# JARVIS-MoCap/JARVIS-HybridNet

Measured on AMD Instinct MI355X. Metric: multi-view frames/s (12cam 1280x1024, 23kpt, 64^3 grid), higher is better.
Workload: dtype f32; 1 GPU; BASELINE configs[2]: HybridNet 12-camera 1280x1024, 23 kpts, 64^3 grid, small/small; cameras=12, joints=23, grid=64, streams=3, parallelism=single GPU, 3 time batches in flight on 3 HIP streams, hipgraph=False

## Files before the change

include/jarvis_hip.h:

```cpp
#ifndef JARVIS_HIP_H
#define JARVIS_HIP_H
#include <stdint.h>

#ifdef __cplusplus
extern "C" {
#endif

#define JH_ABI_VERSION 4

const char* jh_last_error(void);
int jh_abi_version(void);

#define JH_PRECISION_DEFAULT (-1)
#define JH_PRECISION_F32 0
#define JH_PRECISION_BF16X3 1
#define JH_PRECISION_BF16X3_WIDE 2
int jh_set_precision(int mode);
int jh_get_precision(void);

typedef struct jh_params jh_params;
int jh_params_create(jh_params** out);
int jh_params_set(jh_params* p, const char* key, const float* host, int64_t numel);
void jh_params_destroy(jh_params* p);

typedef struct jh_efftrack jh_efftrack;
int jh_efftrack_create(const jh_params* p, const char* prefix, int model_size, int joints, int n,
                       int h, int w, int want_res1, jh_efftrack** out);
int jh_efftrack_forward(jh_efftrack* net, const float* x_dev, float* res1_dev, float* res2_dev,
                        void* stream);
int64_t jh_efftrack_launches(const jh_efftrack* net);
void jh_efftrack_destroy(jh_efftrack* net);

typedef struct jh_v2v jh_v2v;
int jh_v2v_create(const jh_params* p, const char* prefix, int joints, int t, int g, jh_v2v** out);
int jh_v2v_forward(jh_v2v* net, const float* x_dev, float* y_dev, void* stream);
void jh_v2v_destroy(jh_v2v* net);

int64_t jh_reproject_workspace_bytes(int cams, int joints, int hs, int grid_size);
int jh_reproject_forward(const float* heatmaps_padded_dev, int cams, int joints, int hs,
                         const int32_t* center3d_dev, const int32_t* center_hm_dev,
                         const float* cam_dev, const float* intr_dev, const float* dist_dev,
                         int grid_size, float grid_spacing, float* vol_dev, int32_t* idx_dev,
                         void* workspace_dev, int64_t workspace_bytes, void* stream);

int64_t jh_softargmax_workspace_bytes(int t, int joints, int gh);
int jh_softargmax(const float* v2v_out_dev, int t, int joints, int gh, float grid_spacing,
                  float roi_cube_size, const int32_t* center3d_dev, float* heatmap_final_dev,
                  float* points_dev, float* conf_dev, void* workspace_dev, int64_t workspace_bytes,
                  void* stream);

int jh_reproject_point(const float* points_dev, int npoints, int cams, const float* cam_dev,
                       const float* intr_dev, const float* dist_dev, float* uv_dev, void* stream);
int64_t jh_reconstruct_workspace_bytes(int cams);
int jh_reconstruct_point(const float* points2d_dev, const float* maxvals_dev, int cams,
                         const float* cam_dev, const float* intr_dev, const float* dist_dev,
                         float* point3d_dev, void* workspace_dev, int64_t workspace_bytes,
                         void* stream);

typedef struct jh_predictor jh_predictor;
typedef struct {
  int32_t num_cameras, num_joints;
  int32_t center_size;
  int32_t bbox;
  float roi_cube_size;
  float grid_spacing;
  int32_t center_model, kp_model;
  int32_t img_h, img_w;
  int32_t time_batch;
  int32_t time_batch_3d;
  int32_t cam_lo, cam_n;
  float mean[3], std[3];
  int32_t precision;
} jh_predictor_config;

int jh_predictor_create(const jh_params* center_params, const jh_params* hybrid_params,
                        const jh_predictor_config* cfg, jh_predictor** out);
void jh_predictor_destroy(jh_predictor* pr);
int64_t jh_predictor_launches(const jh_predictor* pr);
int64_t jh_predictor_device_bytes(const jh_predictor* pr);
int jh_predictor_precision(const jh_predictor* pr);

int jh_predictor_set_calibration(jh_predictor* pr, const float* cam_dev, const float* intr_dev,
                                 const float* dist_dev, void* stream);
int jh_predictor_set_calibration_frames(jh_predictor* pr, const float* cam_dev ,
                                        const float* intr_dev , const float* dist_dev ,
                                        void* stream);

int jh_predictor_set_centers(jh_predictor* pr, const float* centers_dev , void* stream);

int jh_predictor_stage_center(jh_predictor* pr, const float* frames_dev, float* det_dev,
                              void* stream);
int jh_predictor_stage_keypoints(jh_predictor* pr, const float* frames_dev,
                                 const float* det_all_dev, float* heat_dev, void* stream);
int jh_predictor_stage_3d(jh_predictor* pr, const float* heat_all_dev, int t0, float* points_dev,
                          float* conf_dev, int32_t* valid_dev, void* stream);
int jh_predictor_stage_keypoints_gathered(jh_predictor* pr, const void* frames_dev, int frames_u8,
                                          const float* det_gathered_dev, int n_blocks,
                                          float* heat_dev, void* stream);
int jh_predictor_stage_3d_blocks(jh_predictor* pr, const float* heat_blocks_dev, int n_blocks,
                                 int frames_per_block, int t_off, int t0, float* points_dev,
                                 float* conf_dev, int32_t* valid_dev, void* stream);
int jh_predictor_forward(jh_predictor* pr, const float* frames_dev, float* points_dev,
                         float* conf_dev, int32_t* valid_dev, void* stream);
int jh_predictor_set_graph_replay(jh_predictor* pr, int on);
int jh_predictor_graph_replay(const jh_predictor* pr);
int jh_predictor_stage_center_u8(jh_predictor* pr, const uint8_t* frames_dev, float* det_dev,
                                 void* stream);
int jh_predictor_stage_keypoints_u8(jh_predictor* pr, const uint8_t* frames_dev,
                                    const float* det_all_dev, float* heat_dev, void* stream);
int jh_predictor_forward_u8(jh_predictor* pr, const uint8_t* frames_dev, float* points_dev,
                            float* conf_dev, int32_t* valid_dev, void* stream);

#define JH_FRAME_RGB_F32 0
#define JH_FRAME_BGR_U8 1
#define JH_FRAME_I420 2
#define JH_FRAME_NV12 3
int jh_predictor_forward_yuv(jh_predictor* pr, const uint8_t* frames_dev, int format, float* points_dev,
                             float* conf_dev, int32_t* valid_dev, void* stream);

#define JH_YUV_BT601 0
#define JH_YUV_BT709 1
#define JH_YUV_LIMITED 0
#define JH_YUV_FULL 1
typedef struct jh_yuv_surface {
  int64_t image_stride;
  int64_t y_offset, y_pitch;
  int64_t u_offset, v_offset;
  int64_t c_pitch;
  int32_t c_step;
  int32_t matrix;
  int32_t range;
  int32_t reserved;
} jh_yuv_surface;
int jh_yuv_surface_check(const jh_yuv_surface* surface, int h, int w);
int jh_predictor_forward_surface(jh_predictor* pr, const uint8_t* frames_dev, const jh_yuv_surface* surface,
                                 const uint8_t* mask_dev, float* points_dev, float* conf_dev, int32_t* valid_dev,
                                 void* stream);

#define JH_SENSOR_MONO 0
#define JH_SENSOR_RGGB 1
#define JH_SENSOR_BGGR 2
#define JH_SENSOR_GRBG 3
#define JH_SENSOR_GBRG 4
typedef struct jh_sensor_surface {
  int64_t image_stride;
  int64_t offset, pitch;
  int32_t pattern;
  int32_t reserved;
} jh_sensor_surface;
int jh_sensor_surface_check(const jh_sensor_surface* surface, int h, int w);
int jh_predictor_forward_sensor(jh_predictor* pr, const uint8_t* frames_dev, const jh_sensor_surface* surface,
                                const uint8_t* mask_dev, float* points_dev, float* conf_dev, int32_t* valid_dev,
                                void* stream);

int jh_predictor_debug(jh_predictor* pr, float* center3d_f_dev, int32_t* center3d_i_dev,
                       int32_t* center_hm_dev, float* det_dev, void* stream);

int jh_predictor_forward_masked(jh_predictor* pr, const void* frames_dev, int format, const uint8_t* mask_dev,
                                float* points_dev, float* conf_dev, int32_t* valid_dev, void* stream);
int jh_predictor_stage_keypoints_masked(jh_predictor* pr, const void* frames_dev, int format,
                                        const float* det_all_dev, const uint8_t* mask_dev, float* heat_dev,
                                        void* stream);
int jh_predictor_stage_3d_masked(jh_predictor* pr, const float* heat_all_dev, int t0, const uint8_t* mask_dev,
                                 float* points_dev, float* conf_dev, int32_t* valid_dev, void* stream);
int jh_predictor_debug_mask(jh_predictor* pr, int32_t* n_active_dev, int32_t* num_cams_detect_dev, void* stream);

int jh_predictor_views2d(jh_predictor* pr, const float* heat_all_dev, int t0, const float* points_dev,
                         const uint8_t* mask_dev, int32_t* points2d_dev, float* conf2d_dev, float* reproj_dev,
                         float* err_dev, uint8_t* used_dev, void* stream);

#define JH_FRAME_SURFACE  4
#define JH_FRAME_SENSOR   5
int jh_predictor_forward_images(jh_predictor* pr, const void* const* images_host, int n_images, int format,
                                const jh_yuv_surface* yuv, const jh_sensor_surface* sensor, const uint8_t* mask_dev,
                                float* points_dev, float* conf_dev, int32_t* valid_dev, void* stream);

int jh_predictor_hybridnet_forward(jh_predictor* pr, const float* crops_dev,
                                   const int32_t* center_hm_dev, const int32_t* center3d_dev,
                                   float* heatmap_final_dev, float* heatmaps_padded_dev,
                                   float* points_dev, float* conf_dev, void* stream);

typedef struct jh_predictor2d jh_predictor2d;
int jh_predictor2d_create(const jh_params* center_params, const jh_params* kp_params,
                          const jh_predictor_config* cfg, jh_predictor2d** out);
void jh_predictor2d_destroy(jh_predictor2d* pr);
int jh_predictor2d_forward(jh_predictor2d* pr, const float* frames_dev, int32_t* points_dev,
                           float* conf_dev, int32_t* valid_dev, void* stream);
int jh_predictor2d_forward_u8(jh_predictor2d* pr, const uint8_t* frames_dev, int32_t* points_dev,
                              float* conf_dev, int32_t* valid_dev, void* stream);

int jh_predictor2d_forward_yuv(jh_predictor2d* pr, const uint8_t* frames_dev, int format, int32_t* points_dev,
                               float* conf_dev, int32_t* valid_dev, void* stream);
int jh_predictor2d_forward_surface(jh_predictor2d* pr, const uint8_t* frames_dev, const jh_yuv_surface* surface,
                                   int32_t* points_dev, float* conf_dev, int32_t* valid_dev, void* stream);
int jh_predictor2d_forward_sensor(jh_predictor2d* pr, const uint8_t* frames_dev, const jh_sensor_surface* surface,
                                  int32_t* points_dev, float* conf_dev, int32_t* valid_dev, void* stream);

int jh_predictor2d_forward_images(jh_predictor2d* pr, const void* const* images_host, int n_images, int format,
                                  const jh_yuv_surface* yuv, const jh_sensor_surface* sensor,
                                  int32_t* points_dev, float* conf_dev, int32_t* valid_dev, void* stream);

int jh_profile_begin(void);
int jh_profile_end(int* n_records);
int jh_profile_get(int i, char* name, int name_cap, double* ms, double* flops, double* bytes);

int jh_op_conv(int nd, int kind, int k, int stride, int pad, int cin, int cout,
               const float* w_host, const float* b_host, const float* x_dev, int n, int d, int h,
               int w, const float* gate_dev, int norm_act, float* y_dev, void* stream);
int jh_op_depthwise(int k, int c, const float* w_host, const float* x_dev, int n, int h, int w,
                    int norm_act, float* y_dev, void* stream);
int jh_op_depthwise_pool(int k, int c, const float* w_host, const float* x_dev, int n, int h, int w,
                         float* y_dev, float* pool_dev, void* stream);

int jh_op_yuv420_to_bgr(const uint8_t* frames_dev, int format, int n, int h, int w, uint8_t* out_bgr_dev,
                        void* stream);
int jh_op_yuv_surface_to_bgr(const uint8_t* frames_dev, const jh_yuv_surface* surface, int n, int h, int w,
                             uint8_t* out_bgr_dev, void* stream);
int jh_op_sensor_to_bgr(const uint8_t* frames_dev, const jh_sensor_surface* surface, int n, int h, int w,
                        uint8_t* out_bgr_dev, void* stream);

int64_t jh_joint_argmax_all_workspace_bytes(int n, int hh, int wh, int jp);
int jh_op_joint_argmax_all(const float* heat_dev, int n, int hh, int wh, int j, int jp, int32_t* idx_dev,
                           float* max_dev, void* workspace_dev, int64_t workspace_bytes, void* stream);

int jh_op_bifpn_node(int n_in, const int* modes, const float* weights, int act, int n, int c, int cout,
                     int h, int w, const float* x0_dev, const float* x1_dev, const float* x2_dev,
                     const float* dw_host, const float* pw_host, const float* bias_host, float* y_dev,
                     void* stream);

#ifdef __cplusplus
}
#endif
#endif
```

jarvis-hybridnet_amd/_native.py:

```python
import ctypes
import math
import os
from typing import NamedTuple

import torch

_HERE = os.path.dirname(os.path.abspath(__file__))
LIB_PATH = os.environ.get("JH_LIBRARY_PATH") or os.path.join(_HERE, "libjarvis_hip.so")
_lib = None

c_void_p, c_int, c_float, c_int64 = ctypes.c_void_p, ctypes.c_int, ctypes.c_float, ctypes.c_int64
c_char_p = ctypes.c_char_p


class PredictorConfig(ctypes.Structure):
    _fields_ = [("num_cameras", ctypes.c_int32), ("num_joints", ctypes.c_int32),
                ("center_size", ctypes.c_int32), ("bbox", ctypes.c_int32),
                ("roi_cube_size", c_float), ("grid_spacing", c_float),
                ("center_model", ctypes.c_int32), ("kp_model", ctypes.c_int32),
                ("img_h", ctypes.c_int32), ("img_w", ctypes.c_int32),
                ("time_batch", ctypes.c_int32), ("time_batch_3d", ctypes.c_int32),
                ("cam_lo", ctypes.c_int32),
                ("cam_n", ctypes.c_int32), ("mean", c_float * 3), ("std", c_float * 3),
                ("precision", ctypes.c_int32)]


class YuvSurfaceStruct(ctypes.Structure):
    _fields_ = [("image_stride", ctypes.c_int64), ("y_offset", ctypes.c_int64), ("y_pitch", ctypes.c_int64),
                ("u_offset", ctypes.c_int64), ("v_offset", ctypes.c_int64), ("c_pitch", ctypes.c_int64),
                ("c_step", ctypes.c_int32), ("matrix", ctypes.c_int32), ("range", ctypes.c_int32),
                ("reserved", ctypes.c_int32)]


assert ctypes.sizeof(YuvSurfaceStruct) == 64


class SensorSurfaceStruct(ctypes.Structure):
    _fields_ = [("image_stride", ctypes.c_int64), ("offset", ctypes.c_int64), ("pitch", ctypes.c_int64),
                ("pattern", ctypes.c_int32), ("reserved", ctypes.c_int32)]


assert ctypes.sizeof(SensorSurfaceStruct) == 32

ABI_VERSION = 4
assert ctypes.sizeof(PredictorConfig) == 84

_WORKSPACES = {}


def workspace(nbytes, device):
    key = (str(device), torch.cuda.current_stream(device).cuda_stream)
    bufs = _WORKSPACES.setdefault(key, [])
    if not bufs or bufs[-1].numel() < nbytes:
        bufs.append(torch.empty((max(int(nbytes), 256),), dtype=torch.uint8, device=device))
    return bufs[-1]


_SIGS = {
    "jh_last_error": (c_char_p, []),
    "jh_abi_version": (c_int, []),
    "jh_set_precision": (c_int, [c_int]),
    "jh_get_precision": (c_int, []),
    "jh_params_create": (c_int, [ctypes.POINTER(c_void_p)]),
    "jh_params_set": (c_int, [c_void_p, c_char_p, c_void_p, c_int64]),
    "jh_params_destroy": (None, [c_void_p]),
    "jh_efftrack_create": (c_int, [c_void_p, c_char_p, c_int, c_int, c_int, c_int, c_int, c_int,
                                   ctypes.POINTER(c_void_p)]),
    "jh_efftrack_forward": (c_int, [c_void_p, c_void_p, c_void_p, c_void_p, c_void_p]),
    "jh_efftrack_launches": (c_int64, [c_void_p]),
    "jh_efftrack_destroy": (None, [c_void_p]),
    "jh_v2v_create": (c_int, [c_void_p, c_char_p, c_int, c_int, c_int, ctypes.POINTER(c_void_p)]),
    "jh_v2v_forward": (c_int, [c_void_p, c_void_p, c_void_p, c_void_p]),
    "jh_v2v_destroy": (None, [c_void_p]),
    "jh_reproject_workspace_bytes": (c_int64, [c_int, c_int, c_int, c_int]),
    "jh_reproject_forward": (c_int, [c_void_p, c_int, c_int, c_int, c_void_p, c_void_p, c_void_p,
                                     c_void_p, c_void_p, c_int, c_float, c_void_p, c_void_p,
                                     c_void_p, c_int64, c_void_p]),
    "jh_softargmax_workspace_bytes": (c_int64, [c_int, c_int, c_int]),
    "jh_softargmax": (c_int, [c_void_p, c_int, c_int, c_int, c_float, c_float, c_void_p, c_void_p,
                              c_void_p, c_void_p, c_void_p, c_int64, c_void_p]),
    "jh_reproject_point": (c_int, [c_void_p, c_int, c_int, c_void_p, c_void_p, c_void_p, c_void_p,
                                   c_void_p]),
    "jh_reconstruct_workspace_bytes": (c_int64, [c_int]),
    "jh_reconstruct_point": (c_int, [c_void_p, c_void_p, c_int, c_void_p, c_void_p, c_void_p,
                                     c_void_p, c_void_p, c_int64, c_void_p]),
    "jh_predictor_create": (c_int, [c_void_p, c_void_p, ctypes.POINTER(PredictorConfig),
                                    ctypes.POINTER(c_void_p)]),
    "jh_predictor_destroy": (None, [c_void_p]),
    "jh_predictor_set_graph_replay": (c_int, [c_void_p, c_int]),
    "jh_predictor_graph_replay": (c_int, [c_void_p]),
    "jh_predictor_launches": (c_int64, [c_void_p]),
    "jh_predictor_device_bytes": (c_int64, [c_void_p]),
    "jh_predictor_precision": (c_int, [c_void_p]),
    "jh_predictor_set_calibration": (c_int, [c_void_p, c_void_p, c_void_p, c_void_p, c_void_p]),
    "jh_predictor_set_calibration_frames": (c_int, [c_void_p, c_void_p, c_void_p, c_void_p, c_void_p]),
    "jh_predictor_set_centers": (c_int, [c_void_p, c_void_p, c_void_p]),
    "jh_predictor_stage_center": (c_int, [c_void_p, c_void_p, c_void_p, c_void_p]),
    "jh_predictor_stage_keypoints": (c_int, [c_void_p, c_void_p, c_void_p, c_void_p, c_void_p]),
    "jh_predictor_stage_3d": (c_int, [c_void_p, c_void_p, c_int, c_void_p, c_void_p, c_void_p,
                                      c_void_p]),
    "jh_predictor_stage_keypoints_gathered": (c_int, [c_void_p, c_void_p, c_int, c_void_p, c_int, c_void_p,
                                                      c_void_p]),
    "jh_predictor_stage_3d_blocks": (c_int, [c_void_p, c_void_p, c_int, c_int, c_int, c_int, c_void_p,
                                             c_void_p, c_void_p, c_void_p]),
    "jh_profile_begin": (c_int, []),
    "jh_profile_end": (c_int, [ctypes.POINTER(c_int)]),
    "jh_profile_get": (c_int, [c_int, c_char_p, c_int, ctypes.POINTER(ctypes.c_double),
                               ctypes.POINTER(ctypes.c_double), ctypes.POINTER(ctypes.c_double)]),
    "jh_predictor_forward": (c_int, [c_void_p, c_void_p, c_void_p, c_void_p, c_void_p, c_void_p]),
    "jh_predictor_stage_center_u8": (c_int, [c_void_p, c_void_p, c_void_p, c_void_p]),
    "jh_predictor_stage_keypoints_u8": (c_int, [c_void_p, c_void_p, c_void_p, c_void_p, c_void_p]),
    "jh_predictor_forward_u8": (c_int, [c_void_p, c_void_p, c_void_p, c_void_p, c_void_p, c_void_p]),
    "jh_predictor_forward_yuv": (c_int, [c_void_p, c_void_p, c_int, c_void_p, c_void_p, c_void_p, c_void_p]),
    "jh_yuv_surface_check": (c_int, [ctypes.POINTER(YuvSurfaceStruct), c_int, c_int]),
    "jh_predictor_forward_surface": (c_int, [c_void_p, c_void_p, ctypes.POINTER(YuvSurfaceStruct), c_void_p, c_void_p,
                                             c_void_p, c_void_p, c_void_p]),
    "jh_predictor2d_forward_surface": (c_int, [c_void_p, c_void_p, ctypes.POINTER(YuvSurfaceStruct), c_void_p,
                                               c_void_p, c_void_p, c_void_p]),
    "jh_op_yuv_surface_to_bgr": (c_int, [c_void_p, ctypes.POINTER(YuvSurfaceStruct), c_int, c_int, c_int, c_void_p,
                                         c_void_p]),
    "jh_sensor_surface_check": (c_int, [ctypes.POINTER(SensorSurfaceStruct), c_int, c_int]),
    "jh_predictor_forward_sensor": (c_int, [c_void_p, c_void_p, ctypes.POINTER(SensorSurfaceStruct), c_void_p, c_void_p,
                                            c_void_p, c_void_p, c_void_p]),
    "jh_predictor2d_forward_sensor": (c_int, [c_void_p, c_void_p, ctypes.POINTER(SensorSurfaceStruct), c_void_p,
                                              c_void_p, c_void_p, c_void_p]),
    "jh_op_sensor_to_bgr": (c_int, [c_void_p, ctypes.POINTER(SensorSurfaceStruct), c_int, c_int, c_int, c_void_p,
                                    c_void_p]),
    "jh_predictor_forward_masked": (c_int, [c_void_p, c_void_p, c_int, c_void_p, c_void_p, c_void_p, c_void_p,
                                            c_void_p]),
    "jh_predictor_forward_images": (c_int, [c_void_p, ctypes.POINTER(c_void_p), c_int, c_int,
                                            ctypes.POINTER(YuvSurfaceStruct), ctypes.POINTER(SensorSurfaceStruct),
                                            c_void_p, c_void_p, c_void_p, c_void_p, c_void_p]),
    "jh_predictor2d_forward_images": (c_int, [c_void_p, ctypes.POINTER(c_void_p), c_int, c_int,
                                              ctypes.POINTER(YuvSurfaceStruct), ctypes.POINTER(SensorSurfaceStruct),
                                              c_void_p, c_void_p, c_void_p, c_void_p]),
    "jh_predictor_stage_keypoints_masked": (c_int, [c_void_p, c_void_p, c_int, c_void_p, c_void_p, c_void_p,
                                                    c_void_p]),
    "jh_predictor_stage_3d_masked": (c_int, [c_void_p, c_void_p, c_int, c_void_p, c_void_p, c_void_p, c_void_p,
                                             c_void_p]),
    "jh_predictor_debug_mask": (c_int, [c_void_p, c_void_p, c_void_p, c_void_p]),
    "jh_predictor_views2d": (c_int, [c_void_p, c_void_p, c_int] + [c_void_p] * 8),
    "jh_joint_argmax_all_workspace_bytes": (c_int64, [c_int, c_int, c_int, c_int]),
    "jh_op_joint_argmax_all": (c_int, [c_void_p, c_int, c_int, c_int, c_int, c_int, c_void_p, c_void_p, c_void_p,
                                       c_int64, c_void_p]),
    "jh_predictor2d_create": (c_int, [c_void_p, c_void_p, ctypes.POINTER(PredictorConfig),
                                      ctypes.POINTER(c_void_p)]),
    "jh_predictor2d_destroy": (None, [c_void_p]),
    "jh_predictor2d_forward": (c_int, [c_void_p] * 6),
    "jh_predictor2d_forward_u8": (c_int, [c_void_p] * 6),
    "jh_predictor2d_forward_yuv": (c_int, [c_void_p, c_void_p, c_int, c_void_p, c_void_p, c_void_p, c_void_p]),
    "jh_predictor_debug": (c_int, [c_void_p, c_void_p, c_void_p, c_void_p, c_void_p, c_void_p]),
    "jh_predictor_hybridnet_forward": (c_int, [c_void_p] * 9),
    "jh_op_conv": (c_int, [c_int] * 7 + [c_void_p, c_void_p, c_void_p] + [c_int] * 4 +
                   [c_void_p, c_int, c_void_p, c_void_p]),
    "jh_op_depthwise": (c_int, [c_int, c_int, c_void_p, c_void_p, c_int, c_int, c_int, c_int,
                                c_void_p, c_void_p]),
    "jh_op_depthwise_pool": (c_int, [c_int, c_int, c_void_p, c_void_p, c_int, c_int, c_int, c_void_p, c_void_p,
                                     c_void_p]),
    "jh_op_yuv420_to_bgr": (c_int, [c_void_p, c_int, c_int, c_int, c_int, c_void_p, c_void_p]),
    "jh_op_bifpn_node": (c_int, [c_int, ctypes.POINTER(c_int), ctypes.POINTER(c_float), c_int, c_int, c_int,
                                 c_int, c_int, c_int, c_void_p, c_void_p, c_void_p, c_void_p, c_void_p,
                                 c_void_p, c_void_p, c_void_p]),
}


def symbols():
    return sorted(_SIGS)


def lib():
    global _lib
    if _lib is None:
        if not os.path.isfile(LIB_PATH):
            raise RuntimeError(
                "jarvis_hybridnet_amd: %s is missing -- build it with "
                "`python -c 'import __graft_entry__ as g; g.build()'` (hipcc, gfx950). "
                "There is no CPU fallback." % LIB_PATH)
        handle = ctypes.CDLL(LIB_PATH)
        for name, (res, args) in _SIGS.items():
            fn = getattr(handle, name)
            fn.restype, fn.argtypes = res, args
        if handle.jh_abi_version() != ABI_VERSION:
            raise RuntimeError("libjarvis_hip.so ABI version mismatch")
        _lib = handle
    return _lib


FRAME_CODES = {"rgb": 0, "bgr": 1, "i420": 2, "nv12": 3, "surface": 4, "sensor": 5}
FRAME_FORMATS = {k: FRAME_CODES[k] for k in ("bgr", "i420", "nv12")}
YUV_FORMATS = ("i420", "nv12")
FRAME_SURFACE, FRAME_SENSOR = FRAME_CODES["surface"], FRAME_CODES["sensor"]


class Frames(NamedTuple):
    fmt: int
    height: int
    width: int
    layout: object
    lead: tuple
    data: object = None
    images: object = None

    @property
    def device(self):
        return self.data.device if self.images is None else self.images[0].device


def yuv_format(name):
    if name not in YUV_FORMATS:
        raise ValueError("frame_format must be one of %s, got %r" % (list(YUV_FORMATS), name))
    return name


def surface(layout):
    if layout is None:
        raise ValueError("surface must be a YuvSurface or a SensorSurface, got None")
    return layout


def check_layout(layout, frame_format=None, hw=None):
    if layout is None:
        return None
    from .sensor_surface import SensorSurface
    from .yuv_surface import YuvSurface
    if not isinstance(layout, (YuvSurface, SensorSurface)):
        raise ValueError("frame_layout must be a YuvSurface or a SensorSurface or None, got %r"
                         % (type(layout).__name__,))
    if frame_format in YUV_FORMATS:
        raise ValueError("frame_layout describes the bytes itself: do not combine it with frame_format=%r"
                         % (frame_format,))
    if hw is not None and (layout.height, layout.width) != tuple(hw):
        raise ValueError("frame_layout is %d x %d; this predictor is %d x %d" % (layout.height, layout.width, *hw))
    return layout


def describe_shape(shape, dtype, lead, frame_format=None, frame_layout=None, hw=None, error=ValueError,
                   in_place=False, at_least=False):
    if frame_format is not None and frame_format not in FRAME_FORMATS:
        raise ValueError("frame_format must be one of %s or None, got %r" % (sorted(FRAME_FORMATS), frame_format))
    layout = check_layout(frame_layout, frame_format, hw)
    H, W = hw if hw is not None else ("H", "W")
    hint = ""
    if layout is not None:
        from .sensor_surface import SensorSurface
        kind, error = "sensor" if isinstance(layout, SensorSurface) else "surface", ValueError
        what = "frames of a %s (%simage_stride = %d bytes per image)" % (
            type(layout).__name__, "at least " if at_least else "", layout.image_stride)
        want, tail = torch.uint8, ("image_stride" if at_least else layout.image_stride,)
        H, W = layout.height, layout.width
    elif frame_format in YUV_FORMATS:
        if hw is not None and (H % 2 or W % 2):
            raise ValueError("YUV 4:2:0 frames need an even height and width; this predictor is %d x %d" % (H, W))
        kind, what, want = frame_format, "%s frames" % frame_format, torch.uint8
        tail = (H * 3 // 2, W) if hw is not None else ("3H/2", "W")
    elif dtype == torch.uint8:
        kind, what, want, tail = "bgr", "uint8 BGR frames", torch.uint8, (H, W, 3)
        if shape is not None and len(shape) == len(lead) + 2:
            hint = " (YUV 4:2:0 frames: pass frame_format='i420' or 'nv12')"
    elif frame_format == "bgr":
        raise error("frame_format 'bgr' needs uint8 %s frames; got dtype %s" % (_shape_text(lead, (H, W, 3)), dtype))
    elif dtype == torch.float32 or (not in_place and isinstance(dtype, torch.dtype)):
        kind, what, want, tail = "rgb", "fp32 RGB frames", dtype, (3, H, W)
    else:
        raise error("frames must be float32 RGB %s or uint8 BGR %s; got dtype %s"
                    % (_shape_text(lead, (3, H, W)), _shape_text(lead, (H, W, 3)), dtype))
    full = tuple(lead) + tail
    fits = shape is not None and dtype == want and len(shape) == len(full) and all(
        not isinstance(w, int) or int(g) == w for g, w in zip(shape, full))
    if fits and at_least and layout is not None:
        fits = int(shape[-1]) >= layout.image_stride
    if not fits:
        raise error("%s must be %s of shape %s; got %s%s" % (
            what, "uint8" if want == torch.uint8 else "float32", _shape_text(lead, tail),
            dtype if shape is None else "dtype %s, shape %s" % (dtype, tuple(shape)), hint))
    if kind in YUV_FORMATS and hw is None:
        rows, W = int(shape[-2]), int(shape[-1])
        if rows <= 0 or rows % 3 or W <= 0 or W % 2:
            raise ValueError("a YUV 4:2:0 image is (3H/2, W) bytes with H and W even; got (%d, %d)" % (rows, W))
        H = rows // 3 * 2
    elif hw is None and layout is None:
        H, W = (int(shape[-3]), int(shape[-2])) if kind == "bgr" else (int(shape[-2]), int(shape[-1]))
    return Frames(FRAME_CODES[kind], H, W, layout, tuple(int(n) for n in shape[:len(lead)]))


def _shape_text(lead, tail):
    return "(%s)" % ", ".join("*" if n is None else str(n) for n in tuple(lead) + tuple(tail))


def describe_frames(frames, lead, frame_format=None, frame_layout=None, hw=None, error=ValueError, in_place=False):
    shape, dtype = (frames.shape, frames.dtype) if torch.is_tensor(frames) else (None, type(frames).__name__)
    d = describe_shape(shape, dtype, lead, frame_format, frame_layout, hw, error, in_place)
    if not in_place:
        return d._replace(data=dev(frames, torch.uint8 if d.fmt else torch.float32))
    if not (frames.is_cuda and frames.is_contiguous()):
        raise RuntimeError("frames must be a contiguous CUDA (HIP) tensor")
    return d._replace(data=frames)


def frame_images(images, count, frame_format=None, frame_layout=None):
    lead = (count,) if isinstance(count, int) else tuple(count)
    count = math.prod(lead)
    if not isinstance(images, (list, tuple)) or len(images) != count or not images:
        raise ValueError("expected a sequence of %d images (one tensor per image); got %s" % (
            count, len(images) if isinstance(images, (list, tuple)) else type(images).__name__))
    for i, t in enumerate(images):
        if not torch.is_tensor(t):
            raise ValueError("image %d is a %s, not a tensor" % (i, type(t).__name__))
        if (t.shape, t.dtype, t.device) != (images[0].shape, images[0].dtype, images[0].device):
            raise ValueError("the images of a call have one shape, dtype and device: image %d is %s, image 0 is %s" % (
                i, (t.dtype, tuple(t.shape), str(t.device)),
                (images[0].dtype, tuple(images[0].shape), str(images[0].device))))
    d = describe_shape(images[0].shape, images[0].dtype, (), frame_format, frame_layout, in_place=True, at_least=True)
    for i, t in enumerate(images):
        if not t.is_contiguous():
            raise RuntimeError("image %d is not contiguous: the kernels read it in place" % i)
        if not t.is_cuda:
            raise RuntimeError("jarvis_hybridnet_amd needs CUDA (HIP) tensors; image %d is a CPU tensor" % i)
    return d._replace(lead=lead, images=list(images))


def forward_symbol(which, fmt, masked=False, per_image=False):
    if per_image:
        return which + "_forward_images"
    if fmt in (FRAME_SURFACE, FRAME_SENSOR):
        return which + ("_forward_surface" if fmt == FRAME_SURFACE else "_forward_sensor")
    if masked:
        return which + "_forward_masked"
    return which + ("_forward", "_forward_u8", "_forward_yuv", "_forward_yuv")[fmt]


def call_forward(which, handle, frames, mask, outs):
    masks = which == "jh_predictor"
    if mask is not None and not masks:
        raise ValueError("%s takes no camera mask" % which)
    name = forward_symbol(which, frames.fmt, mask is not None, frames.images is not None)
    struct = frames.layout.struct() if frames.layout is not None else None
    if frames.images is not None:
        table = (c_void_p * len(frames.images))(*(t.data_ptr() for t in frames.images))
        args = (table, len(frames.images), frames.fmt, struct if frames.fmt == FRAME_SURFACE else None,
                struct if frames.fmt == FRAME_SENSOR else None) + ((ptr(mask),) if masks else ())
    elif struct is not None:
        args = (ptr(frames.data), struct) + ((ptr(mask),) if masks else ())
    elif mask is not None:
        args = (ptr(frames.data), frames.fmt, ptr(mask))
    else:
        args = (ptr(frames.data),) + ((frames.fmt,) if frames.fmt >= FRAME_CODES["i420"] else ())
    check(getattr(lib(), name)(handle, *args, *(ptr(t) for t in outs), stream()))


def camera_mask(mask, shape, what="camera_mask"):
    if mask is None:
        return None
    if not torch.is_tensor(mask):
        try:
            mask = torch.as_tensor(mask)
        except Exception as e:
            raise ValueError("%s must be a bool or integer tensor or sequence of shape %s: %s" % (what, tuple(shape), e))
    if mask.dtype.is_floating_point or mask.dtype.is_complex:
        raise ValueError("%s must be bool or integer (nonzero = use the camera); got dtype %s" % (what, mask.dtype))
    if tuple(mask.shape) != tuple(shape):
        raise ValueError("%s must have shape %s; got %s" % (what, tuple(shape), tuple(mask.shape)))
    return (mask != 0).to(torch.uint8).contiguous()


_CALIB_TAILS = ((4, 3), (3, 3), (1, 5))


def calibration(calib, T, C):
    if not isinstance(calib, (list, tuple)) or len(calib) != 3 or not all(torch.is_tensor(t) for t in calib):
        raise ValueError("calibration is three tensors (cameraMatrices, intrinsicMatrices, distortionCoefficients); "
                         "got %s" % ([type(t).__name__ for t in calib] if isinstance(calib, (list, tuple))
                                     else type(calib).__name__))
    names = ("cameraMatrices", "intrinsicMatrices", "distortionCoefficients")
    forms = []
    for name, t, tail in zip(names, calib, _CALIB_TAILS):
        if not t.dtype.is_floating_point:
            raise ValueError("%s must be a floating-point tensor; got dtype %s" % (name, t.dtype))
        shape = tuple(int(n) for n in t.shape)
        if shape == (C,) + tail:
            forms.append("shared")
        elif shape == (T, C) + tail:
            forms.append("frames")
        else:
            raise ValueError("%s must have shape %s (shared by the frame sets) or %s (one per frame set); got %s"
                             % (name, (C,) + tail, (T, C) + tail, shape))
    if len(set(forms)) != 1:
        raise ValueError("the three calibration tensors are either all per camera (C, ...) or all per frame set "
                         "(T, C, ...); got %s" % ", ".join("%s: %s" % nf for nf in zip(names, forms)))
    return (forms[0],) + tuple(calib)


def centers(value, T):
    if value is None:
        return None
    want = "(%d, 3)" % T + (" or (3,)" if T == 1 else "")
    if not torch.is_tensor(value):
        try:
            value = torch.as_tensor(value)
        except Exception as e:
            raise ValueError("centers must be a real numeric tensor, array or sequence of shape %s: %s" % (want, e))
    if value.dtype == torch.bool or value.dtype.is_complex:
        raise ValueError("centers must have a real numeric dtype; got %s" % value.dtype)
    shape = tuple(int(n) for n in value.shape)
    if shape == (3,) and T == 1:
        value = value.unsqueeze(0)
    elif shape != (T, 3):
        raise ValueError("centers must have shape %s (world millimetres, one row per frame set); got %s" % (want, shape))
    return value.to(torch.float32).contiguous()


PRECISIONS = {"f32": 0, "bf16x3": 1, "bf16x3_wide": 2}
PRECISION_DEFAULT = -1


def precision_id(mode):
    if mode is None:
        return PRECISION_DEFAULT
    if mode not in PRECISIONS:
        raise ValueError("precision must be one of %s or None, got %r" % (sorted(PRECISIONS), mode))
    return PRECISIONS[mode]


def set_precision(mode):
    prev = get_precision()
    check(lib().jh_set_precision(PRECISIONS[mode]))
    return prev


def get_precision():
    return {v: k for k, v in PRECISIONS.items()}[lib().jh_get_precision()]


def check(rc):
    if rc != 0:
        raise RuntimeError("libjarvis_hip: " + lib().jh_last_error().decode())


def ptr(t):
    if t is None:
        return None
    assert t.is_contiguous(), "tensor must be contiguous"
    return t.data_ptr()


def dev(t, dtype=torch.float32):
    if not t.is_cuda:
        raise RuntimeError("jarvis_hybridnet_amd needs CUDA (HIP) tensors; got a CPU tensor")
    return t.to(dtype).contiguous()


def stream():
    return torch.cuda.current_stream().cuda_stream


class Params:

    def __init__(self, state_dict):
# ... 29 lines not shown
```

jarvis-hybridnet_amd/csrc/api.hip:

```cpp
#include <cstring>
#include <memory>
#include "../../include/jarvis_hip.h"
#include <cstdlib>
#include "nets.h"
#include "bifpn_node.h"
#include "camera_mask.h"
#include "views2d.h"

namespace jh {
static thread_local std::string g_err;
void set_error(const std::string& msg) { g_err = msg; }
}

using namespace jh;

struct jh_params { ParamMap map; };
struct jh_efftrack { EffTrackPlan plan; };
struct jh_v2v { V2VPlan plan; };

namespace {

struct Scratch {
  std::vector<void*> ptrs;
  ~Scratch() { for (void* p : ptrs) (void)hipFree(p); }
// ... 818 lines not shown
  return forward_impl(pr, frames_dev, fixed_source(kSrcBgrU8), points_dev, conf_dev, valid_dev, stream);
}

int jh_predictor_forward_yuv(jh_predictor* pr, const uint8_t* frames_dev, int format, float* points_dev,
                             float* conf_dev, int32_t* valid_dev, void* stream) {
  JH_REQUIRE(format == JH_FRAME_I420 || format == JH_FRAME_NV12, "jh_predictor_forward_yuv: format must be "
             "JH_FRAME_I420 or JH_FRAME_NV12");
  JH_REQUIRE(pr, "bad argument");
  FrameSource fs;
  if (frame_source(format, pr->cfg.img_h, pr->cfg.img_w, &fs)) return 1;
  return forward_impl(pr, frames_dev, fs, points_dev, conf_dev, valid_dev, stream);
}

int jh_yuv_surface_check(const jh_yuv_surface* surface, int h, int w) { return yuv_surface_check(surface, h, w); }

int jh_predictor_forward_surface(jh_predictor* pr, const uint8_t* frames_dev, const jh_yuv_surface* surface,
                                 const uint8_t* mask_dev, float* points_dev, float* conf_dev, int32_t* valid_dev,
                                 void* stream) {
  JH_REQUIRE(pr, "bad argument");
  FrameSource fs;
  if (frame_source(surface, pr->cfg.img_h, pr->cfg.img_w, &fs)) return 1;
  return forward_impl(pr, frames_dev, fs, points_dev, conf_dev, valid_dev, stream, mask_dev);
}

int jh_sensor_surface_check(const jh_sensor_surface* surface, int h, int w) {
  return sensor_surface_check(surface, h, w);
}

int jh_predictor_forward_sensor(jh_predictor* pr, const uint8_t* frames_dev, const jh_sensor_surface* surface,
                                const uint8_t* mask_dev, float* points_dev, float* conf_dev, int32_t* valid_dev,
                                void* stream) {
  JH_REQUIRE(pr, "bad argument");
  FrameSource fs;
  if (frame_source(surface, pr->cfg.img_h, pr->cfg.img_w, &fs)) return 1;
  return forward_impl(pr, frames_dev, fs, points_dev, conf_dev, valid_dev, stream, mask_dev);
}

int jh_predictor_forward_masked(jh_predictor* pr, const void* frames_dev, int format, const uint8_t* mask_dev,
                                float* points_dev, float* conf_dev, int32_t* valid_dev, void* stream) {
  JH_REQUIRE(pr, "bad argument");
  JH_REQUIRE(format >= JH_FRAME_RGB_F32 && format <= JH_FRAME_NV12, "jh_predictor_forward_masked: unknown frame format");
  FrameSource fs;
  if (frame_source(format, pr->cfg.img_h, pr->cfg.img_w, &fs)) return 1;
  return forward_impl(pr, frames_dev, fs, points_dev, conf_dev, valid_dev, stream, mask_dev);
}

int jh_predictor_forward_images(jh_predictor* pr, const void* const* images_host, int n_images, int format,
                                const jh_yuv_surface* yuv, const jh_sensor_surface* sensor, const uint8_t* mask_dev,
                                float* points_dev, float* conf_dev, int32_t* valid_dev, void* stream) {
  JH_REQUIRE(pr, "bad argument");
  JH_REQUIRE(pr->Cloc == pr->C && pr->cfg.cam_lo == 0, "forward needs all cameras local");
  FrameSource fs;
  if (images_source(format, yuv, sensor, pr->cfg.img_h, pr->cfg.img_w, &fs)) return 1;
  if (upload_images(pr->mem, &pr->frames_table, images_host, n_images, pr->T * pr->C, format,
                    static_cast<hipStream_t>(stream))) return 1;
  return forward_impl(pr, pr->frames_table, fs, points_dev, conf_dev, valid_dev, stream, mask_dev);
}

int jh_predictor_stage_keypoints_masked(jh_predictor* pr, const void* frames_dev, int format,
                                        const float* det_all_dev, const uint8_t* mask_dev, float* heat_dev,
                                        void* stream) {
  JH_REQUIRE(pr && mask_dev, "bad argument");
  JH_REQUIRE(format == JH_FRAME_RGB_F32 || format == JH_FRAME_BGR_U8, "masked stage 2: fp32 RGB or uint8 BGR frames");
  JH_REQUIRE(pr->Cloc == pr->C && pr->cfg.cam_lo == 0, "masked stage 2 needs all cameras local");
  pr->mask_cur = mask_dev;
  const int rc = stage_keypoints_impl(pr, frames_dev, fixed_source(format), det_all_dev, heat_dev, stream, 1, true);
  pr->mask_cur = nullptr;
  return rc;
}

int jh_predictor_stage_3d_masked(jh_predictor* pr, const float* heat_all_dev, int t0, const uint8_t* mask_dev,
                                 float* points_dev, float* conf_dev, int32_t* valid_dev, void* stream) {
  JH_REQUIRE(pr && mask_dev, "bad argument");
  JH_REQUIRE(pr->Cloc == pr->C && pr->cfg.cam_lo == 0, "masked stage 3 needs all cameras local");
  pr->mask_cur = mask_dev;
  const int rc = jh_predictor_stage_3d(pr, heat_all_dev, t0, points_dev, conf_dev, valid_dev, stream);
  pr->mask_cur = nullptr;
  return rc;
}

int jh_predictor_debug_mask(jh_predictor* pr, int32_t* n_active_dev, int32_t* num_cams_detect_dev, void* stream) {
  hipStream_t s = static_cast<hipStream_t>(stream);
  JH_REQUIRE(pr, "bad argument");
  const size_t T = pr->T;
  if (n_active_dev) JH_CHECK_HIP(hipMemcpyAsync(n_active_dev, pr->n_active, T * sizeof(int), hipMemcpyDeviceToDevice, s));
  if (num_cams_detect_dev) JH_CHECK_HIP(hipMemcpyAsync(num_cams_detect_dev, pr->n_detect, T * sizeof(int), hipMemcpyDeviceToDevice, s));
  return 0;
}

int jh_predictor_views2d(jh_predictor* pr, const float* heat_all_dev, int t0, const float* points_dev,
                         const uint8_t* mask_dev, int32_t* points2d_dev, float* conf2d_dev, float* reproj_dev,
                         float* err_dev, uint8_t* used_dev, void* stream) {
  hipStream_t s = static_cast<hipStream_t>(stream);
  JH_REQUIRE(pr && points_dev && points2d_dev && conf2d_dev && reproj_dev && err_dev && used_dev,
             "null pointer");
  JH_REQUIRE(t0 >= 0 && t0 + pr->T3 <= pr->T, "frame range of the 2D views");
  const int N = pr->T3 * pr->C;
  if (!heat_all_dev) {
    JH_REQUIRE(pr->Cloc == pr->C && pr->cfg.cam_lo == 0, "the predictor's own heat maps hold all cameras only when "
               "all cameras are local");
    heat_all_dev = pr->kp->heat.p + (size_t)t0 * pr->C * pr->Hh * pr->Hh * pr->Jp;
  }
  if (!pr->v2d_max) {
    hipStreamCaptureStatus cs = hipStreamCaptureStatusNone;
    (void)hipStreamIsCapturing(s, &cs);
    JH_REQUIRE(cs == hipStreamCaptureStatusNone, "the first jh_predictor_views2d call of a predictor allocates its "
               "workspace: make it outside a stream capture");
    const size_t n = joint_argmax_all_partials(N, pr->Hh, pr->Hh, pr->Jp);
    if (pr->mem.get(reinterpret_cast<void**>(&pr->v2d_max), n * sizeof(float))) return 1;
    if (pr->mem.get(reinterpret_cast<void**>(&pr->v2d_idx), n * sizeof(int))) return 1;
  }
  const double bytes = 4.0 * N * pr->Hh * pr->Hh * pr->Jp;
  JH_PROF("joint_argmax_all", 0.0, bytes,
          launch_joint_argmax_all(heat_all_dev, pr->v2d_max, pr->v2d_idx, N, pr->Hh, pr->Hh, pr->J, pr->Jp, s));
  const int slices = joint_argmax_all_shape(N, pr->Hh, pr->Hh, pr->Jp).slices;
  JH_PROF("views2d_final", 0.0, 8.0 * N * slices * pr->Jp + 24.0 * N * pr->J,
          launch_views2d_final(pr->v2d_max, pr->v2d_idx, pr->chm_cur() + (size_t)t0 * pr->C * 2, pr->valid_cur() + t0,
                               mask_dev ? mask_dev + (size_t)t0 * pr->C : nullptr, points_dev, pr->cam_at(t0),
                               pr->intr_at(t0), pr->dist_at(t0), pr->calib_fs, points2d_dev, conf2d_dev, reproj_dev,
                               err_dev, used_dev, pr->T3, pr->C,
                               pr->J, pr->Jp, pr->Hh, pr->Hh, pr->B / 2, s));
  return 0;
}

int jh_predictor_debug(jh_predictor* pr, float* center3d_f_dev, int32_t* center3d_i_dev,
                       int32_t* center_hm_dev, float* det_dev, void* stream) {
  hipStream_t s = static_cast<hipStream_t>(stream);
  const size_t T = pr->T, C = pr->C;
  if (center3d_f_dev) JH_CHECK_HIP(hipMemcpyAsync(center3d_f_dev, pr->c3f, T * 3 * sizeof(float), hipMemcpyDeviceToDevice, s));
  if (center3d_i_dev) JH_CHECK_HIP(hipMemcpyAsync(center3d_i_dev, pr->c3i_cur(), T * 3 * sizeof(int), hipMemcpyDeviceToDevice, s));
  if (center_hm_dev) JH_CHECK_HIP(hipMemcpyAsync(center_hm_dev, pr->chm_cur(), T * C * 2 * sizeof(int), hipMemcpyDeviceToDevice, s));
  if (det_dev) JH_CHECK_HIP(hipMemcpyAsync(det_dev, pr->det_all, T * C * 3 * sizeof(float), hipMemcpyDeviceToDevice, s));
  return 0;
}

int jh_predictor_hybridnet_forward(jh_predictor* pr, const float* crops_dev,
                                   const int32_t* center_hm_dev, const int32_t* center3d_dev,
                                   float* heatmap_final_dev, float* heatmaps_padded_dev,
                                   float* points_dev, float* conf_dev, void* stream) {
  hipStream_t s = static_cast<hipStream_t>(stream);
  JH_REQUIRE(pr->Cloc == pr->C && pr->T3 == pr->T, "hybridnet_forward needs all cameras local");
  JH_CHECK_HIP(hipMemcpyAsync(pr->chm_cur(), center_hm_dev, (size_t)pr->T * pr->C * 2 * sizeof(int), hipMemcpyDeviceToDevice, s));
  JH_CHECK_HIP(hipMemcpyAsync(pr->c3i_cur(), center3d_dev, (size_t)pr->T * 3 * sizeof(int), hipMemcpyDeviceToDevice, s));
  if (launch_to_channel_last(crops_dev, pr->kp->input, s)) return 1;
  pr->kp->stem_src.mode = 0;
  if (pr->kp->run(s)) return 1;
  if (heatmaps_padded_dev) {
    const Act& h = pr->kp->heat;
    const size_t total = (size_t)h.N * pr->J * pr->hs * pr->hs;
    int blocks = (int)((total + 255) / 256);
    if (blocks > 8192) blocks = 8192;
    hipLaunchKernelGGL(export_padded_kernel, dim3(blocks), dim3(256), 0, s, h.p, heatmaps_padded_dev,
                       h.N, pr->J, h.Cp, pr->Hh);
    JH_CHECK_HIP(hipGetLastError());
  }
  return pr->run_3d(pr->kp->heat.p, 0, heatmap_final_dev, points_dev, conf_dev, s);
}

}

struct jh_predictor2d {
  jh_predictor_config cfg{};
  int T = 0, J = 0, B = 0;
  std::unique_ptr<EffTrackPlan> center, kp;
  Scratch mem;
  float* det = nullptr;
  int *chm = nullptr, *valid = nullptr;
  const void** frames_table = nullptr;
};

extern "C" {

int jh_predictor2d_create(const jh_params* center_params, const jh_params* kp_params,
                          const jh_predictor_config* cfg, jh_predictor2d** out) {
  JH_REQUIRE(center_params && kp_params && cfg && out, "bad argument");
  std::unique_ptr<jh_predictor2d> pr(new jh_predictor2d());
  pr->cfg = *cfg;
  pr->T = cfg->time_batch; pr->J = cfg->num_joints; pr->B = cfg->bbox;
  JH_REQUIRE(pr->T >= 1, "batch");
  JH_REQUIRE(cfg->img_w >= pr->B + 1 && cfg->img_h >= pr->B + 1, "image smaller than the bounding box");
  JH_REQUIRE(cfg->precision >= JH_PRECISION_DEFAULT && cfg->precision <= JH_PRECISION_BF16X3_WIDE,
             "jh_predictor_config.precision: unknown mode");
  const int precision = cfg->precision == JH_PRECISION_DEFAULT ? precision_mode() : cfg->precision;
  pr->cfg.precision = precision;
  pr->center.reset(new EffTrackPlan());
  pr->center->precision = precision;
  if (pr->center->build(center_params->map, "", cfg->center_model, 1, pr->T, cfg->center_size,
                        cfg->center_size)) return 1;
  pr->kp.reset(new EffTrackPlan());
  pr->kp->precision = precision;
  if (pr->kp->build(kp_params->map, "", cfg->kp_model, pr->J, pr->T, pr->B, pr->B)) return 1;
  if (pr->mem.get(reinterpret_cast<void**>(&pr->det), (size_t)pr->T * 3 * sizeof(float))) return 1;
  if (pr->mem.get(reinterpret_cast<void**>(&pr->chm), (size_t)pr->T * 2 * sizeof(int))) return 1;
  if (pr->mem.get(reinterpret_cast<void**>(&pr->valid), (size_t)pr->T * sizeof(int))) return 1;
  JH_CHECK_HIP(hipDeviceSynchronize());
  *out = pr.release();
  return 0;
}

void jh_predictor2d_destroy(jh_predictor2d* pr) { delete pr; }

static int forward2d_impl(jh_predictor2d* pr, const void* frames, const FrameSource& fs, int32_t* points_dev,
                          float* conf_dev, int32_t* valid_dev, void* stream) {
  hipStream_t s = static_cast<hipStream_t>(stream);
  const auto& c = pr->cfg;
  const int S = c.center_size;
  JH_PROF("preprocess_resize", 0.0, (double)pr->T * S * S * (4.0 * fs.px_bytes() + 12.0),
          launch_preprocess_resize(frames, fs, pr->center->input.p, pr->T, c.img_h, c.img_w, S,
                                   c.mean, c.std, s, fs.per_image ? pr->frames_table : nullptr));
  if (pr->center->run(s)) return 1;
  const Act& h = pr->center->heat;
  JH_PROF("center_argmax", 0.0, 4.0 * pr->T * h.H * h.W,
          launch_center_argmax(h.p, pr->det, pr->T, h.H, h.W, h.Cp, s));
  const float sx = (float)c.img_w / (float)S, sy = (float)c.img_h / (float)S;
  if (launch_center2d(pr->det, pr->chm, pr->valid, pr->T, sx, sy, pr->B / 2, c.img_w, c.img_h, s))
    return 1;
  JH_PROF("preprocess_crop", 0.0, (double)pr->T * pr->B * pr->B * (fs.px_bytes() + 12.0),
          launch_preprocess_crop(frames, fs, pr->chm, pr->kp->input.p, pr->T, 1, 1, 0, c.img_h,
                                 c.img_w, pr->B, c.mean, c.std, s, fs.per_image ? pr->frames_table : nullptr));
  if (pr->kp->run(s)) return 1;
  const Act& k = pr->kp->heat;
  JH_PROF("joint_argmax", 0.0, 4.0 * pr->T * k.H * k.W * pr->J,
          launch_joint_argmax(k.p, pr->chm, points_dev, conf_dev, pr->T, pr->J, k.Cp, k.H, k.W,
                              pr->B / 2, s));
  if (valid_dev)
    JH_CHECK_HIP(hipMemcpyAsync(valid_dev, pr->valid, (size_t)pr->T * sizeof(int),
                                hipMemcpyDeviceToDevice, s));
  return 0;
}

int jh_predictor2d_forward(jh_predictor2d* pr, const float* frames_dev, int32_t* points_dev,
                           float* conf_dev, int32_t* valid_dev, void* stream) {
  return forward2d_impl(pr, frames_dev, fixed_source(kSrcRgbF32), points_dev, conf_dev, valid_dev, stream);
}
int jh_predictor2d_forward_u8(jh_predictor2d* pr, const uint8_t* frames_dev, int32_t* points_dev,
                              float* conf_dev, int32_t* valid_dev, void* stream) {
  return forward2d_impl(pr, frames_dev, fixed_source(kSrcBgrU8), points_dev, conf_dev, valid_dev, stream);
}

int jh_predictor2d_forward_yuv(jh_predictor2d* pr, const uint8_t* frames_dev, int format, int32_t* points_dev,
                               float* conf_dev, int32_t* valid_dev, void* stream) {
  JH_REQUIRE(format == JH_FRAME_I420 || format == JH_FRAME_NV12, "jh_predictor2d_forward_yuv: format must be "
             "JH_FRAME_I420 or JH_FRAME_NV12");
  JH_REQUIRE(pr, "bad argument");
  FrameSource fs;
  if (frame_source(format, pr->cfg.img_h, pr->cfg.img_w, &fs)) return 1;
  return forward2d_impl(pr, frames_dev, fs, points_dev, conf_dev, valid_dev, stream);
}

int jh_predictor2d_forward_surface(jh_predictor2d* pr, const uint8_t* frames_dev, const jh_yuv_surface* surface,
                                   int32_t* points_dev, float* conf_dev, int32_t* valid_dev, void* stream) {
  JH_REQUIRE(pr && frames_dev, "bad argument");
  FrameSource fs;
  if (frame_source(surface, pr->cfg.img_h, pr->cfg.img_w, &fs)) return 1;
  return forward2d_impl(pr, frames_dev, fs, points_dev, conf_dev, valid_dev, stream);
}

int jh_predictor2d_forward_sensor(jh_predictor2d* pr, const uint8_t* frames_dev, const jh_sensor_surface* surface,
                                  int32_t* points_dev, float* conf_dev, int32_t* valid_dev, void* stream) {
  JH_REQUIRE(pr && frames_dev, "bad argument");
  FrameSource fs;
  if (frame_source(surface, pr->cfg.img_h, pr->cfg.img_w, &fs)) return 1;
  return forward2d_impl(pr, frames_dev, fs, points_dev, conf_dev, valid_dev, stream);
}

int jh_predictor2d_forward_images(jh_predictor2d* pr, const void* const* images_host, int n_images, int format,
                                  const jh_yuv_surface* yuv, const jh_sensor_surface* sensor,
                                  int32_t* points_dev, float* conf_dev, int32_t* valid_dev, void* stream) {
  JH_REQUIRE(pr && points_dev && conf_dev, "bad argument");
  FrameSource fs;
  if (images_source(format, yuv, sensor, pr->cfg.img_h, pr->cfg.img_w, &fs)) return 1;
  if (upload_images(pr->mem, &pr->frames_table, images_host, n_images, pr->T, format,
                    static_cast<hipStream_t>(stream))) return 1;
  return forward2d_impl(pr, pr->frames_table, fs, points_dev, conf_dev, valid_dev, stream);
}

int jh_profile_begin(void) {
  Profiler& pf = profiler();
  pf.recs.clear();
  pf.on = true;
  return 0;
}
int jh_profile_end(int* n_records) {
  Profiler& pf = profiler();
  pf.on = false;
  if (pf.finish()) return 1;
  if (n_records) *n_records = (int)pf.recs.size();
  return 0;
}
int jh_profile_get(int i, char* name, int name_cap, double* ms, double* flops, double* bytes) {
  Profiler& pf = profiler();
  JH_REQUIRE(i >= 0 && i < (int)pf.recs.size(), "profile record index");
  const ProfRec& r = pf.recs[i];
  if (name && name_cap > 0) {
    strncpy(name, r.name.c_str(), name_cap - 1);
    name[name_cap - 1] = 0;
  }
  if (ms) *ms = r.ms;
  if (flops) *flops = r.flops;
  if (bytes) *bytes = r.bytes;
  return 0;
}

int jh_op_conv(int nd, int kind, int k, int stride, int pad, int cin, int cout,
               const float* w_host, const float* b_host, const float* x_dev, int n, int d, int h,
               int w, const float* gate_dev, int norm_act, float* y_dev, void* stream) {
  hipStream_t s = static_cast<hipStream_t>(stream);
  ConvDesc desc = kind == 0 ? conv_desc(nd, k, stride, pad, cin, cout)
                            : (kind == 1 ? deconv2d_k4s2p1_desc(cin, cout) : deconv3d_k2s2_desc(cin, cout));
  Scratch sc;
  Act x, y;
  if (nd == 2) d = 1;
  if (sc.act(n, d, h, w, cin, &x)) return 1;
  int Do, Ho, Wo;
  conv_out_shape(desc, d, h, w, &Do, &Ho, &Wo);
  if (sc.act(n, Do, Ho, Wo, cout, &y)) return 1;
  JH_CHECK_HIP(hipMemsetAsync(y.p, 0, y.bytes(), s));
  bool wino = kind == 0 && nd == 3 && k == 3 && stride == 1 && pad == 1 && !gate_dev;
  if (const char* e = getenv("JH_WINO")) wino = wino && atoi(e) != 0;
  const bool b3 = wino && precision_mode() >= 1;
  const bool d4b = kind == 1 && !b_host && norm_act < 0 && !gate_dev && precision_mode() >= 1 &&
                   deconv4_bf16x3_eligible(cout);
  const bool xb = kind == 0 && !wino && !gate_dev && conv_bf16x3_eligible(desc) && x.Cp == cpad(cin) &&
                  (precision_mode() == 2 || (precision_mode() == 1 && nd == 3));
  ConvWeights cw;
  if (xb) {
    if (pack_conv_bf16x3_weights(desc, w_host, b_host, &cw)) return 1;
  } else if (d4b) {
    if (pack_deconv4_bf16x3_weights(cin, cout, w_host, &cw)) return 1;
  } else if (b3) {
    if (pack_bf16x3_weights(cin, cout, w_host, b_host, &cw)) return 1;
  } else if (wino) {
    if (pack_wino_weights(cin, cout, w_host, b_host, &cw)) return 1;
  } else {
    if (pack_conv_weights(desc, w_host, b_host, kind != 0, &cw)) return 1;
  }
  double* stats = nullptr;
  float* gate_p = nullptr;
  int rc = 0;
  do {
    if (norm_act >= 0) {
      if ((rc = sc.get(reinterpret_cast<void**>(&stats), (size_t)n * y.Cp * kStatW * sizeof(double)))) break;
      if (hipMemsetAsync(stats, 0, (size_t)n * y.Cp * kStatW * sizeof(double), s) != hipSuccess) { rc = 1; break; }
    }
    if (gate_dev) {
      if ((rc = sc.get(reinterpret_cast<void**>(&gate_p), (size_t)n * x.Cp * sizeof(float)))) break;
      if (hipMemsetAsync(gate_p, 0, (size_t)n * x.Cp * sizeof(float), s) != hipSuccess) { rc = 1; break; }
      if (hipMemcpy2DAsync(gate_p, x.Cp * sizeof(float), gate_dev, cin * sizeof(float),
                           cin * sizeof(float), n, hipMemcpyDeviceToDevice, s) != hipSuccess) { rc = 1; break; }
    }
    if ((rc = launch_to_channel_last(x_dev, x, s))) break;
    if (xb) { if ((rc = launch_conv_bf16x3(desc, cw, x, y, stats, s, nullptr))) break; }
    else if (d4b) { if ((rc = launch_deconv4_bf16x3(cw, x, y, s, nullptr))) break; }
    else if (b3) { if ((rc = launch_conv3d_bf16x3(cw, x, y, stats, s, nullptr))) break; }
    else if (wino) { if ((rc = launch_conv3d_wino(cw, x, y, stats, s, nullptr, wino_variant_from_env()))) break; }
    else if ((rc = launch_conv(desc, cw, x, y, gate_p, stats, s))) break;
    if (norm_act >= 0 && (rc = launch_norm_apply(y, stats, 1e-5, norm_act, nullptr, nullptr, y.p, nullptr, s))) break;
    if ((rc = launch_from_channel_last(y, y_dev, s))) break;
    if (hipStreamSynchronize(s) != hipSuccess) { set_error("stream sync failed in jh_op_conv"); rc = 1; }
  } while (0);
  free_conv_weights(&cw);
  return rc;
}

int jh_op_depthwise(int k, int c, const float* w_host, const float* x_dev, int n, int h, int w,
                    int norm_act, float* y_dev, void* stream) {
  hipStream_t s = static_cast<hipStream_t>(stream);
  Scratch sc;
  Act x, y;
  if (sc.act(n, 1, h, w, c, &x)) return 1;
  if (sc.act(n, 1, h, w, c, &y)) return 1;
  std::vector<float> wt((size_t)k * k * x.Cp, 0.f);
  for (int ch = 0; ch < c; ++ch)
    for (int t = 0; t < k * k; ++t) wt[(size_t)t * x.Cp + ch] = w_host[(size_t)ch * k * k + t];
  float* wd; double* stats = nullptr;
  if (sc.get(reinterpret_cast<void**>(&wd), wt.size() * sizeof(float))) return 1;
  JH_CHECK_HIP(hipMemcpyAsync(wd, wt.data(), wt.size() * sizeof(float), hipMemcpyHostToDevice, s));
  if (norm_act >= 0) {
    if (sc.get(reinterpret_cast<void**>(&stats), (size_t)n * x.Cp * kStatW * sizeof(double))) return 1;
    JH_CHECK_HIP(hipMemsetAsync(stats, 0, (size_t)n * x.Cp * kStatW * sizeof(double), s));
  }
  if (launch_to_channel_last(x_dev, x, s)) return 1;
  if (launch_depthwise(x, wd, k, y.p, stats, s)) return 1;
  if (norm_act >= 0 && launch_norm_apply(y, stats, 1e-5, norm_act, nullptr, nullptr, y.p, nullptr, s)) return 1;
  if (launch_from_channel_last(y, y_dev, s)) return 1;
  JH_CHECK_HIP(hipStreamSynchronize(s));
  return 0;
}

int jh_op_yuv420_to_bgr(const uint8_t* frames_dev, int format, int n, int h, int w, uint8_t* out_bgr_dev,
                        void* stream) {
  hipStream_t s = static_cast<hipStream_t>(stream);
  JH_REQUIRE(frames_dev && out_bgr_dev, "null frame / output pointer");
  JH_REQUIRE(format == JH_FRAME_I420 || format == JH_FRAME_NV12, "jh_op_yuv420_to_bgr: format must be "
             "JH_FRAME_I420 or JH_FRAME_NV12");
  FrameSource fs;
  if (frame_source(format, h, w, &fs) || launch_frames_to_bgr(frames_dev, fs, out_bgr_dev, n, h, w, s)) return 1;
  JH_CHECK_HIP(hipStreamSynchronize(s));
  return 0;
}

int jh_op_yuv_surface_to_bgr(const uint8_t* frames_dev, const jh_yuv_surface* surface, int n, int h, int w,
                             uint8_t* out_bgr_dev, void* stream) {
  hipStream_t s = static_cast<hipStream_t>(stream);
  JH_REQUIRE(frames_dev && out_bgr_dev && n >= 1, "null frame / output pointer");
  FrameSource fs;
  if (frame_source(surface, h, w, &fs) || launch_frames_to_bgr(frames_dev, fs, out_bgr_dev, n, h, w, s)) return 1;
  JH_CHECK_HIP(hipStreamSynchronize(s));
  return 0;
}

int jh_op_sensor_to_bgr(const uint8_t* frames_dev, const jh_sensor_surface* surface, int n, int h, int w,
                        uint8_t* out_bgr_dev, void* stream) {
  hipStream_t s = static_cast<hipStream_t>(stream);
  JH_REQUIRE(frames_dev && out_bgr_dev && n >= 1, "null frame / output pointer");
  FrameSource fs;
  if (frame_source(surface, h, w, &fs) || launch_frames_to_bgr(frames_dev, fs, out_bgr_dev, n, h, w, s)) return 1;
  JH_CHECK_HIP(hipStreamSynchronize(s));
  return 0;
}

int jh_op_depthwise_pool(int k, int c, const float* w_host, const float* x_dev, int n, int h, int w,
                         float* y_dev, float* pool_dev, void* stream) {
  hipStream_t s = static_cast<hipStream_t>(stream);
  JH_REQUIRE(depthwise_can_pool(h, w), "jh_op_depthwise_pool: the image must be one 16 x 16 tile");
  Scratch sc;
  Act x, y;
  if (sc.act(n, 1, h, w, c, &x)) return 1;
  if (sc.act(n, 1, h, w, c, &y)) return 1;
  std::vector<float> wt((size_t)k * k * x.Cp, 0.f);
  for (int ch = 0; ch < c; ++ch)
    for (int t = 0; t < k * k; ++t) wt[(size_t)t * x.Cp + ch] = w_host[(size_t)ch * k * k + t];
  float* wd; double *stats = nullptr, *pool = nullptr;
  if (sc.get(reinterpret_cast<void**>(&wd), wt.size() * sizeof(float))) return 1;
  JH_CHECK_HIP(hipMemcpyAsync(wd, wt.data(), wt.size() * sizeof(float), hipMemcpyHostToDevice, s));
  const size_t nst = (size_t)n * x.Cp * kStatW, npl = (size_t)n * x.Cp * kLimbs;
  if (sc.get(reinterpret_cast<void**>(&stats), nst * sizeof(double))) return 1;
  if (sc.get(reinterpret_cast<void**>(&pool), npl * sizeof(double))) return 1;
  JH_CHECK_HIP(hipMemsetAsync(stats, 0, nst * sizeof(double), s));
  JH_CHECK_HIP(hipMemsetAsync(pool, 0, npl * sizeof(double), s));
  if (launch_to_channel_last(x_dev, x, s)) return 1;
  if (launch_depthwise(x, wd, k, y.p, stats, s, pool)) return 1;
  if (launch_from_channel_last(y, y_dev, s)) return 1;
  std::vector<double> hp(npl);
  JH_CHECK_HIP(hipMemcpyAsync(hp.data(), pool, npl * sizeof(double), hipMemcpyDeviceToHost, s));
  JH_CHECK_HIP(hipStreamSynchronize(s));
  std::vector<float> out((size_t)n * c);
  for (int i = 0; i < n; ++i)
    for (int ch = 0; ch < c; ++ch) {
      const double* q = hp.data() + ((size_t)i * x.Cp + ch) * kLimbs;
      out[(size_t)i * c + ch] = (float)((q[0] + q[1]) + q[2]);
    }
  JH_CHECK_HIP(hipMemcpy(pool_dev, out.data(), out.size() * sizeof(float), hipMemcpyHostToDevice));
  return 0;
}

static size_t carve_joint_argmax_all(Carver& c, int n, int hh, int wh, int jp, float** pmax, int** pidx) {
  const size_t k = joint_argmax_all_partials(n, hh, wh, jp);
  *pmax = c.take<float>(k);
  *pidx = c.take<int>(k);
  return c.off;
}

int64_t jh_joint_argmax_all_workspace_bytes(int n, int hh, int wh, int jp) {
  if (n < 1 || hh < 1 || wh < 1 || jp < 8 || jp % 8 || jp > 256) return 0;
  Carver c(nullptr, 0);
  float* pmax;
  int* pidx;
  return (int64_t)carve_joint_argmax_all(c, n, hh, wh, jp, &pmax, &pidx);
}

int jh_op_joint_argmax_all(const float* heat_dev, int n, int hh, int wh, int j, int jp, int32_t* idx_dev,
                           float* max_dev, void* workspace_dev, int64_t workspace_bytes, void* stream) {
  hipStream_t s = static_cast<hipStream_t>(stream);
  JH_REQUIRE(heat_dev && idx_dev && max_dev, "null pointer");
  JH_REQUIRE(n >= 1 && hh >= 1 && wh >= 1 && jp >= 8 && jp % 8 == 0 && jp <= 256 && j >= 1 && j <= jp,
             "jh_op_joint_argmax_all: shape");
  JH_REQUIRE(workspace_dev && workspace_bytes >= 0, "workspace (see jh_joint_argmax_all_workspace_bytes)");
  Carver c(workspace_dev, (size_t)workspace_bytes);
  float* pmax;
  int* pidx;
  carve_joint_argmax_all(c, n, hh, wh, jp, &pmax, &pidx);
  JH_REQUIRE(c.fits(), "workspace smaller than jh_joint_argmax_all_workspace_bytes()");
  const double bytes = 4.0 * n * hh * wh * jp;
  JH_PROF("joint_argmax_all", 0.0, bytes, launch_joint_argmax_all(heat_dev, pmax, pidx, n, hh, wh, j, jp, s));
  if (launch_joint_argmax_all_combine(pmax, pidx, idx_dev, max_dev, n, hh, wh, j, jp, s)) return 1;
  JH_CHECK_HIP(hipStreamSynchronize(s));
  return 0;
}


int jh_op_bifpn_node(int n_in, const int* modes, const float* weights, int act, int n, int c, int cout,
                     int h, int w, const float* x0_dev, const float* x1_dev, const float* x2_dev,
                     const float* dw_host, const float* pw_host, const float* bias_host, float* y_dev,
                     void* stream) {
  hipStream_t s = static_cast<hipStream_t>(stream);
  JH_REQUIRE(n_in >= 2 && n_in <= 3 && modes && weights && y_dev, "bad argument");
  const float* xs[3] = {x0_dev, x1_dev, x2_dev};
  Scratch sc;
  Act in[3], y;
  NodeArgs a{};
  a.n_in = n_in; a.act = act;
  for (int i = 0; i < n_in; ++i) {
    int hi = h, wi = w;
    if (modes[i] == FUSE_UP2) { hi = h / 2; wi = w / 2; }
    else if (modes[i] == FUSE_UP4) { hi = h / 4; wi = w / 4; }
    else if (modes[i] == FUSE_POOL2) { hi = h * 2; wi = w * 2; }
    if (sc.act(n, 1, hi, wi, c, &in[i])) return 1;
    if (launch_to_channel_last(xs[i], in[i], s)) return 1;
    const size_t px = (size_t)hi * wi;
    std::vector<float> host((size_t)n * c * px);
    JH_CHECK_HIP(hipMemcpyAsync(host.data(), xs[i], host.size() * sizeof(float), hipMemcpyDeviceToHost, s));
    JH_CHECK_HIP(hipStreamSynchronize(s));
    std::vector<double> st((size_t)n * in[i].Cp * kStatW, 0.0);
    for (int b = 0; b < n; ++b)
      for (int ch = 0; ch < c; ++ch) {
        double s1 = 0.0, s2 = 0.0;
        const float* p = host.data() + ((size_t)b * c + ch) * px;
        for (size_t k = 0; k < px; ++k) { s1 += p[k]; s2 += (double)p[k] * p[k]; }
        st[((size_t)b * in[i].Cp + ch) * kStatW + 1] = s1;
        st[((size_t)b * in[i].Cp + ch) * kStatW + kLimbs + 1] = s2;
      }
    double* std_dev;
    if (sc.get(reinterpret_cast<void**>(&std_dev), st.size() * sizeof(double))) return 1;
    JH_CHECK_HIP(hipMemcpyAsync(std_dev, st.data(), st.size() * sizeof(double), hipMemcpyHostToDevice, s));
    JH_CHECK_HIP(hipStreamSynchronize(s));
    a.in[i] = in[i].p; a.st[i] = std_dev; a.inv_cnt[i] = 1.f / (float)px; a.mode[i] = modes[i];
    a.w[i] = weights[i];
  }
  if (sc.act(n, 1, h, w, cout, &y)) return 1;
  JH_CHECK_HIP(hipMemsetAsync(y.p, 0, y.bytes(), s));
  const int Cp = in[0].Cp;
  std::vector<float> dwt((size_t)9 * Cp, 0.f);
  for (int ch = 0; ch < c; ++ch)
    for (int t = 0; t < 9; ++t) dwt[(size_t)t * Cp + ch] = dw_host[(size_t)ch * 9 + t];
  float* dwd;
  if (sc.get(reinterpret_cast<void**>(&dwd), dwt.size() * sizeof(float))) return 1;
  JH_CHECK_HIP(hipMemcpyAsync(dwd, dwt.data(), dwt.size() * sizeof(float), hipMemcpyHostToDevice, s));
  ConvWeights cw;
  if (pack_conv_weights(conv_desc(2, 1, 1, 0, c, cout), pw_host, bias_host, false, &cw)) return 1;
  double* ost;
  int rc = 0;
  do {
    if ((rc = sc.get(reinterpret_cast<void**>(&ost), (size_t)n * y.Cp * kStatW * sizeof(double)))) break;
    if (hipMemsetAsync(ost, 0, (size_t)n * y.Cp * kStatW * sizeof(double), s) != hipSuccess) { rc = 1; break; }
    a.dw = dwd; a.pw = cw.w; a.bias = cw.bias; a.y = y.p; a.stats = ost;
    a.N = n; a.H = h; a.W = w; a.Cp = Cp; a.cout_p = y.Cp; a.cout_p16 = cw.cout_p16;
    if ((rc = launch_bifpn_node(a, s))) break;
    if ((rc = launch_from_channel_last(y, y_dev, s))) break;
    if (hipStreamSynchronize(s) != hipSuccess) { set_error("stream sync failed in jh_op_bifpn_node"); rc = 1; }
  } while (0);
  free_conv_weights(&cw);
  return rc;
}

}
```

jarvis-hybridnet_amd/csrc/conv_host.hip:

```cpp
#include <vector>
#include <cstring>
#include <cstdlib>
#include <algorithm>
#include "conv_mfma.h"

namespace jh {

ConvDesc conv_desc(int nd, int k, int stride, int pad, int cin, int cout) {
  ConvDesc d{};
  d.nd = nd; d.k = k; d.stride = stride; d.ostride = 1; d.nphase = 1;
  d.cin = cin; d.cout = cout;
  d.phase[0].pad[0] = (nd == 3) ? pad : 0;
  d.phase[0].pad[1] = pad; d.phase[0].pad[2] = pad;
  d.phase[0].ooff[0] = d.phase[0].ooff[1] = d.phase[0].ooff[2] = 0;
  return d;
}

ConvDesc deconv2d_k4s2p1_desc(int cin, int cout) {
  ConvDesc d{};
  d.nd = 2; d.k = 2; d.stride = 1; d.ostride = 2; d.nphase = 4;
  d.cin = cin; d.cout = cout;
  for (int py = 0; py < 2; ++py)
    for (int px = 0; px < 2; ++px) {
      ConvPhase& p = d.phase[py * 2 + px];
      p.pad[0] = 0; p.pad[1] = py ? 0 : 1; p.pad[2] = px ? 0 : 1;
      p.ooff[0] = 0; p.ooff[1] = py; p.ooff[2] = px;
    }
  return d;
}

ConvDesc deconv3d_k2s2_desc(int cin, int cout) {
  ConvDesc d{};
  d.nd = 3; d.k = 1; d.stride = 1; d.ostride = 2; d.nphase = 8;
  d.cin = cin; d.cout = cout;
  for (int p = 0; p < 8; ++p) {
    d.phase[p].pad[0] = d.phase[p].pad[1] = d.phase[p].pad[2] = 0;
    d.phase[p].ooff[0] = (p >> 2) & 1; d.phase[p].ooff[1] = (p >> 1) & 1; d.phase[p].ooff[2] = p & 1;
  }
  return d;
}

void conv_out_shape(const ConvDesc& d, int D, int H, int W, int* Do, int* Ho, int* Wo) {
  if (d.ostride > 1) {
    *Do = (d.nd == 3) ? D * d.ostride : 1; *Ho = H * d.ostride; *Wo = W * d.ostride;
    return;
  }
  const int kd = (d.nd == 3) ? d.k : 1;
  *Do = (d.nd == 3) ? (D + 2 * d.phase[0].pad[0] - kd) / d.stride + 1 : 1;
  *Ho = (H + 2 * d.phase[0].pad[1] - d.k) / d.stride + 1;
  *Wo = (W + 2 * d.phase[0].pad[2] - d.k) / d.stride + 1;
}

static inline int deconv4_tap(int parity, int t) { return parity ? (t == 0 ? 2 : 0) : (t == 0 ? 3 : 1); }

int pack_conv_weights(const ConvDesc& d, const float* w, const float* b, bool transposed,
                      ConvWeights* out) {
  const int cin_p = cpad(d.cin);
  const int cout_p16 = round_up(d.cout, 16);
  const int kd = (d.nd == 3) ? d.k : 1;
  const int ntap = kd * d.k * d.k;
  const int nk8 = cin_p / 8, nb = cout_p16 / 16;
  const size_t phase_stride = (size_t)ntap * nk8 * nb * 128;
  std::vector<float> packed(phase_stride * d.nphase, 0.f);
  const bool paired = d.nd == 2 && d.ostride > 1 && deconv4_eligible(cin_p, cout_p16);
  const bool tap_paired = d.nd == 3 && d.k == 3 && d.stride == 2 && d.ostride == 1;
  if (tap_paired) packed.assign((size_t)((ntap + 1) / 2) * nk8 * nb * 256, 0.f);
  int skd, sk;
  if (d.ostride > 1 && d.nd == 2) { skd = 1; sk = 4; }
  else if (d.ostride > 1 && d.nd == 3) { skd = 2; sk = 2; }
  else { skd = kd; sk = d.k; }
  const size_t sktaps = (size_t)skd * sk * sk;
  for (int ph = 0; ph < d.nphase; ++ph) {
    for (int tz = 0; tz < kd; ++tz)
      for (int ty = 0; ty < d.k; ++ty)
        for (int tx = 0; tx < d.k; ++tx) {
          int sz = tz, sy = ty, sx = tx;
          if (d.ostride > 1 && d.nd == 2) {
            sy = deconv4_tap(d.phase[ph].ooff[1], ty);
            sx = deconv4_tap(d.phase[ph].ooff[2], tx);
          } else if (d.ostride > 1 && d.nd == 3) {
            sz = d.phase[ph].ooff[0]; sy = d.phase[ph].ooff[1]; sx = d.phase[ph].ooff[2];
          }
          const size_t stap = ((size_t)sz * sk + sy) * sk + sx;
          const int tap = (tz * d.k + ty) * d.k + tx;
          for (int ci = 0; ci < d.cin; ++ci)
            for (int co = 0; co < d.cout; ++co) {
              const float v = transposed ? w[((size_t)ci * d.cout + co) * sktaps + stap]
                                         : w[((size_t)co * d.cin + ci) * sktaps + stap];
              const int kc8 = ci / 8, kq = (ci % 8) / 2, j = ci % 2;
              const int nbk = co / 16, nn = co % 16;
              const int lane = kq * 16 + nn;
              if (tap_paired)
                packed[((((size_t)(tap / 2)) * nk8 + kc8) * nb + nbk) * 256 + lane * 4 + (tap & 1) * 2 + j] = v;
              else if (paired)
                packed[ph * phase_stride + (((size_t)tap * (nk8 / 2) + kc8 / 2) * nb + nbk) * 256 + lane * 4 + (kc8 & 1) * 2 + j] = v;
              else
                packed[ph * phase_stride + (((size_t)tap * nk8 + kc8) * nb + nbk) * 128 + lane * 2 + j] = v;
            }
        }
  }
  out->cin_p = cin_p; out->cout_p16 = cout_p16; out->paired = tap_paired ? 2 : (paired ? 1 : 0);
  out->phase_stride = tap_paired ? packed.size() : phase_stride;
  JH_CHECK_HIP(hipMalloc(&out->w, packed.size() * sizeof(float)));
  JH_CHECK_HIP(hipMemcpy(out->w, packed.data(), packed.size() * sizeof(float), hipMemcpyHostToDevice));
  out->bias = nullptr;
  if (b) {
    std::vector<float> bp(cout_p16, 0.f);
    std::memcpy(bp.data(), b, d.cout * sizeof(float));
    JH_CHECK_HIP(hipMalloc(&out->bias, bp.size() * sizeof(float)));
    JH_CHECK_HIP(hipMemcpy(out->bias, bp.data(), bp.size() * sizeof(float), hipMemcpyHostToDevice));
  }
  return 0;
}

void free_conv_weights(ConvWeights* w) {
  if (w->w) (void)hipFree(w->w);
  if (w->bias) (void)hipFree(w->bias);
  w->w = w->bias = nullptr;
}

static int pick_nr(int nb, int taps, bool heavy_staging, long units) {
  const double stage = (heavy_staging ? 1.5 : 0.5) / (double)taps;
  const long slots = 512;
  int best = 1;
  double best_cost = 1e30;
  for (int nr = 4; nr >= 1; --nr) {
    const long groups = (nb + nr - 1) / nr;
    const double cost = (double)std::max(units * groups, slots) * (stage + nr);
    if (cost < best_cost - 1e-9) { best_cost = cost; best = nr; }
  }
  return best;
}

int launch_conv(const ConvDesc& d, const ConvWeights& w, const Act& x, const Act& y,
                const float* gate, double* stats, hipStream_t s, const InNorm* in, const SeGate* se) {
  JH_REQUIRE(x.Cp == w.cin_p || (x.Cp == 4 && w.cin_p == 8), "conv input channel padding mismatch");
  JH_REQUIRE(y.Cp == cpad(d.cout), "conv output channel padding mismatch");
  JH_REQUIRE(x.N == y.N, "batch mismatch");
  ConvArgs a{};
  a.x = x.p; a.y = y.p; a.w = w.w; a.bias = w.bias; a.gate = gate; a.stats = stats;
  if (in && in->stats) {
    a.in_stats = in->stats; a.in_inv = in->inv; a.in_act = in->act;
    a.nrm_floats = 2 * w.cin_p;
  }
  if (gate) a.nrm_floats += w.cin_p;
  if (se && se->pool) {
    JH_REQUIRE(!gate, "either a gate tensor or a gate recipe");
    a.se = *se;
    a.nrm_floats += w.cin_p + round_up(se->C, 4) + round_up(se->S, 4);
  }
  a.N = x.N; a.Din = x.D; a.Hin = x.H; a.Win = x.W; a.cin_p = w.cin_p; a.in_px = x.Cp;
  a.Dy = y.D; a.Hy = y.H; a.Wy = y.W; a.cout_p = y.Cp; a.cout_p16 = w.cout_p16;
  a.ostride = d.ostride; a.nphase = d.nphase; a.phase_stride = w.phase_stride; a.paired = w.paired;
  for (int p = 0; p < d.nphase; ++p) a.phase[p] = d.phase[p];
  if (d.ostride > 1) { a.Dout = x.D; a.Hout = x.H; a.Wout = x.W; }
  else conv_out_shape(d, x.D, x.H, x.W, &a.Dout, &a.Hout, &a.Wout);
  int Do, Ho, Wo;
  conv_out_shape(d, x.D, x.H, x.W, &Do, &Ho, &Wo);
  JH_REQUIRE(Do == y.D && Ho == y.H && Wo == y.W, "conv output extent mismatch");
  const int taps = d.k * d.k * (d.nd == 3 ? d.k : 1);
  long units;
  if (d.nd == 2) units = (long)((a.Hout + 7) / 8) * ((a.Wout <= 8 ? a.Wout + 7 : a.Wout + 15) / (a.Wout <= 8 ? 8 : 16));
  else units = (long)((a.Dout + 1) / 2) * ((a.Hout + 3) / 4) * ((a.Wout + 15) / 16);
  units *= (long)a.nphase * a.N;
  const int nr = pick_nr(w.cout_p16 / 16, taps, (in && in->stats && in->act == ACT_SILU) || gate || (se && se->pool),
                         units);
  const size_t budget = 40 * 1024;
  if (d.nd == 2 && d.ostride == 2 && d.k == 2) {
    const int rc = launch_deconv4_fused(a, s);
    if (rc >= 0) return rc;
  }
  JH_REQUIRE((a.paired == 2) == (d.nd == 3 && d.k == 3 && d.stride == 2 && d.ostride == 1) && a.paired != 1,
             "paired weight layout without a kernel that reads it");
  if (conv_pw_direct_eligible(d, a)) return launch_conv_pw_direct(a, s);
  if (d.nd == 2) {
    const int small = (a.Wout <= 8) ? 1 : 0;
    const int big = (a.Wout >= 64 && a.Hout >= 64 && w.cin_p <= 32 && d.ostride == 1 && d.stride == 1 &&
               (d.k == 1 || d.k == 3)) ? 1 : 0;
    if (big) return conv_launch_2d_big(a, d.k, d.stride, nr, budget, s);
    if (d.k == 1 && d.stride == 1 && d.ostride == 1 && d.nphase == 1 && (a.Wout % 16 != 0 || a.Hout % 8 != 0) &&
        a.Hout * a.Wout >= 96 && a.Hin == a.Hout && a.Win == a.Wout && a.Hy == a.Hout && a.Wy == a.Wout) {
      ConvArgs f = a;
      f.Win = f.Wout = f.Wy = a.Hout * a.Wout;
      f.Hin = f.Hout = f.Hy = 1;
      return conv_launch_2d_k1_flat(f, nr, budget, s);
    }
    if (d.k == 1 && d.stride == 1) return conv_launch_2d_k1(a, nr, small, budget, s);
    if (d.k == 2 && d.stride == 1) return conv_launch_2d_k2(a, nr, small, budget, s);
    if (d.k == 3 && d.stride == 1 && d.ostride == 1 && a.Wout > 16 && a.Wout <= 20 && a.Hout <= 22 &&
        !d.latency_class)
      return conv_launch_2d_k3_w20(a, nr, std::max(budget, (size_t)64 * 1024), s);
    if (!d.latency_class && d.ostride == 1) {
      if (d.k == 5 && d.stride <= 2 && a.Wout > 32 && a.Wout <= 40)
        return conv_launch_2d_k5_w40(a, d.stride, nr, std::max(budget, (size_t)64 * 1024), s);
      if (d.k == 3 && d.stride == 2 && a.Wout > 16 && a.Wout <= 20 && a.Hout <= 22)
        return conv_launch_2d_k3s2_w20(a, nr, std::max(budget, (size_t)96 * 1024), s);
    }
    if (d.k == 3 && d.stride <= 2) return conv_launch_2d_k3(a, d.stride, nr, small, budget, s);
    if (d.k == 5 && d.stride <= 2) return conv_launch_2d_k5(a, d.stride, nr, small, budget, s);
  } else {
    const int nr_form = pick_nr(w.cout_p16 / 16, taps,
                                (in && in->stats && in->act == ACT_SILU) || gate || (se && se->pool), 1L << 40);
    const long tiles_big = (long)((a.Dout + 1) / 2) * ((a.Hout + 3) / 4) * ((a.Wout + 15) / 16) *
                           a.nphase * ((w.cout_p16 / 16 + nr_form - 1) / nr_form);
    int small = tiles_big < 16 ? 1 : 0;
    if (!small && d.k == 3 && d.stride == 1 && tiles_big >= 256) small = 2;
    if (d.k == 1 && d.stride == 1) return conv_launch_3d_k1(a, nr, small, budget, s);
    if (d.k == 2 && d.stride == 2) return conv_launch_3d_k2s2(a, nr, small, budget, s);
    if (d.k == 3 && d.stride <= 2) return conv_launch_3d_k3(a, d.stride, nr, small, budget, s);
  }
  JH_REQUIRE(false, "no convolution kernel for this (nd, k, stride)");
}

}
```

jarvis-hybridnet_amd/csrc/conv_mfma.h:

```cpp
#pragma once
#include <cstdlib>
#include <type_traits>
#include "jh_common.h"

namespace jh {

typedef float f32x4 __attribute__((ext_vector_type(4)));

template <int ND, int K, int STRIDE, int TZ, int TY, int TX>
struct ConvGeom {
  static constexpr int KD = (ND == 3) ? K : 1;
  static constexpr int KH = K, KW = K;
  static constexpr int NT = KD * KH * KW;
  static constexpr int PZ = (TZ - 1) * STRIDE + KD;
  static constexpr int PY = (TY - 1) * STRIDE + KH;
  static constexpr int PX = (TX - 1) * STRIDE + KW;
  static constexpr int NPIX = PZ * PY * PX;
  static constexpr int TM = TZ * TY * TX;
  static constexpr int MR = TM / 64;
  static constexpr int SPAD = (STRIDE == 1) ? 4 : 2;
  static_assert(TM % 64 == 0 || (TZ == 1 && TM / 64 >= 1), "tile must cover at least 64 pixels");
  static size_t lds_bytes(int kc) { return (size_t)NPIX * (kc + SPAD) * sizeof(float); }
};

// ... 280 lines not shown
      const float4 mu = *reinterpret_cast<const float4*>(nrm + c);
      const float4 rs = *reinterpret_cast<const float4*>(nrm + a.cin_p + c);
      v.x = (v.x - mu.x) * rs.x; v.y = (v.y - mu.y) * rs.y;
      v.z = (v.z - mu.z) * rs.z; v.w = (v.w - mu.w) * rs.w;
      if (a.in_act == ACT_RELU) {
        v.x = fmaxf(v.x, 0.f); v.y = fmaxf(v.y, 0.f); v.z = fmaxf(v.z, 0.f); v.w = fmaxf(v.w, 0.f);
      } else if (a.in_act == ACT_SILU) {
        v.x = silu_fast(v.x); v.y = silu_fast(v.y);
        v.z = silu_fast(v.z); v.w = silu_fast(v.w);
      }
    }
    if (gated) {
      const float4 g = *reinterpret_cast<const float4*>(gate_l + c);
      v.x *= g.x; v.y *= g.y; v.z *= g.z; v.w *= g.w;
    }
    return v;
  };
  if constexpr (PF) issue_pf(0);

  constexpr bool TAPPAIR = ND == 3 && K == 3 && STRIDE == 2;
  constexpr bool PIPE = (G::NT > 1) && (MR * NR * KC8 >= 12) && !TAPPAIR;
  constexpr bool BREG = !PIPE && (G::NT == 1 ? KC8 * NR <= 16 : G::NT * KC8 * NR <= 9);
  for (int c0 = 0; c0 < a.cin_p; c0 += KC) {
    float2 breg[BREG ? G::NT : 1][KC8][NR];
    if constexpr (BREG) {
#pragma unroll
      for (int tp = 0; tp < G::NT; ++tp)
#pragma unroll
        for (int k8 = 0; k8 < KC8; ++k8)
#pragma unroll
          for (int nr = 0; nr < NR; ++nr)
            breg[tp][k8][nr] = wload(tp * tap_stride + min((c0 >> 3) + k8, nkc8_total - 1) * nb16_total * 64, nr);
    }
    __syncthreads();
    if constexpr (PF) {
      const int mode = !a.in_stats ? 0 : (a.in_act == ACT_RELU ? 2 : (a.in_act == ACT_SILU ? 3 : 1));
      auto commit_pf = [&](auto mode_c) __attribute__((always_inline)) {
        constexpr int MODE = decltype(mode_c)::value;
        float4 mu0 = make_float4(0.f, 0.f, 0.f, 0.f), rs0 = make_float4(1.f, 1.f, 1.f, 1.f), gt0 = rs0;
        if (CQ) {
          const int cc = min(c0 + (tid % Q4) * 4, a.cin_p - 4);
          if (MODE != 0) {
            mu0 = *reinterpret_cast<const float4*>(nrm + cc);
            rs0 = *reinterpret_cast<const float4*>(nrm + a.cin_p + cc);
          }
          if (gated) gt0 = *reinterpret_cast<const float4*>(gate_l + cc);
        }
#pragma unroll
        for (int it = 0; it < ITER; ++it) {
          const int idx = tid + it * 256;
          if (idx < G::NPIX * Q4) {
            const int c4 = idx % Q4, pix = idx / Q4;
            float4 mu = mu0, rs = rs0, gt = gt0;
            if (!CQ) {
              const int cc = min(c0 + c4 * 4, a.cin_p - 4);
              if (MODE != 0) {
                mu = *reinterpret_cast<const float4*>(nrm + cc);
                rs = *reinterpret_cast<const float4*>(nrm + a.cin_p + cc);
              }
              if (gated) gt = *reinterpret_cast<const float4*>(gate_l + cc);
            }
            float4 v = pf[it];
            if (MODE != 0) {
              const float m = (pvo[it] < 0 || c0 + c4 * 4 >= a.in_px) ? 0.f : 1.f;
              v.x = (v.x - mu.x) * rs.x; v.y = (v.y - mu.y) * rs.y;
              v.z = (v.z - mu.z) * rs.z; v.w = (v.w - mu.w) * rs.w;
              if (MODE == 2) {
                v.x = fmaxf(v.x, 0.f); v.y = fmaxf(v.y, 0.f); v.z = fmaxf(v.z, 0.f); v.w = fmaxf(v.w, 0.f);
              } else if (MODE == 3) {
                v.x = silu_fast(v.x); v.y = silu_fast(v.y);
                v.z = silu_fast(v.z); v.w = silu_fast(v.w);
              }
              v.x *= m; v.y *= m; v.z *= m; v.w *= m;
            }
            if (gated) { v.x *= gt.x; v.y *= gt.y; v.z *= gt.z; v.w *= gt.w; }
            float2* dst = lds2 + pix * S2 + c4 * 2;
            dst[0] = make_float2(v.x, v.y);
            dst[1] = make_float2(v.z, v.w);
          }
        }
      };
      if (mode == 0) commit_pf(std::integral_constant<int, 0>{});
      else if (mode == 3) commit_pf(std::integral_constant<int, 3>{});
      else if (mode == 2) commit_pf(std::integral_constant<int, 2>{});
      else commit_pf(std::integral_constant<int, 1>{});
    } else {
      for (int idx = tid; idx < G::NPIX * Q4; idx += 256) {
        const float* src;
        const bool ok = patch_ok(idx, c0, &src);
        const int c4 = idx % Q4, pix = idx / Q4;
        float4 v = make_float4(0.f, 0.f, 0.f, 0.f);
        if (ok) v = finish(*reinterpret_cast<const float4*>(src), c0 + c4 * 4);
        float2* dst = lds2 + pix * S2 + c4 * 2;
        dst[0] = make_float2(v.x, v.y);
        dst[1] = make_float2(v.z, v.w);
      }
    }
    __syncthreads();
    if constexpr (PF) {
      if (c0 + KC < a.cin_p) issue_pf(c0 + KC);
    }

    if constexpr (PIPE) {
      int koff[KC8];
#pragma unroll
      for (int k8 = 0; k8 < KC8; ++k8)
        koff[k8] = min((c0 >> 3) + k8, nkc8_total - 1) * nb16_total * 64;
      float2 bn[KC8][NR], an[KC8][MR];
#pragma unroll
      for (int k8 = 0; k8 < KC8; ++k8) {
#pragma unroll
        for (int nr = 0; nr < NR; ++nr) bn[k8][nr] = wload(koff[k8], nr);
#pragma unroll
        for (int mr = 0; mr < MR; ++mr) an[k8][mr] = lds2[abase[mr] + k8 * 4];
      }
      for (int row = 0; row < G::KD * G::KH; ++row) {
        const int dz = row / G::KH, dy = row % G::KH;
        const int row_off = (dz * G::PY + dy) * G::PX * S2;
        const int nrow = min(row + 1, G::KD * G::KH - 1);
        const int next_row_off = ((nrow / G::KH) * G::PY + nrow % G::KH) * G::PX * S2;
#pragma unroll
        for (int dx = 0; dx < G::KW; ++dx) {
          const int tap = row * G::KW + dx;
          float2 bc[KC8][NR], ac[KC8][MR];
#pragma unroll
          for (int k8 = 0; k8 < KC8; ++k8) {
#pragma unroll
            for (int mr = 0; mr < MR; ++mr) ac[k8][mr] = an[k8][mr];
#pragma unroll
            for (int nr = 0; nr < NR; ++nr) bc[k8][nr] = bn[k8][nr];
          }
          const int wn = min(tap + 1, G::NT - 1) * tap_stride;
          const int noff = (dx + 1 < G::KW) ? row_off + (dx + 1) * S2 : next_row_off;
#pragma unroll
          for (int k8 = 0; k8 < KC8; ++k8) {
#pragma unroll
            for (int nr = 0; nr < NR; ++nr) bn[k8][nr] = wload(wn + koff[k8], nr);
#pragma unroll
            for (int mr = 0; mr < MR; ++mr) an[k8][mr] = lds2[abase[mr] + noff + k8 * 4];
          }
#pragma unroll
          for (int k8 = 0; k8 < KC8; ++k8) {
#pragma unroll
            for (int mr = 0; mr < MR; ++mr)
#pragma unroll
              for (int nr = 0; nr < NR; ++nr)
                acc[mr][nr] = __builtin_amdgcn_mfma_f32_16x16x4f32(ac[k8][mr].x, bc[k8][nr].x, acc[mr][nr], 0, 0, 0);
#pragma unroll
            for (int mr = 0; mr < MR; ++mr)
#pragma unroll
              for (int nr = 0; nr < NR; ++nr)
                acc[mr][nr] = __builtin_amdgcn_mfma_f32_16x16x4f32(ac[k8][mr].y, bc[k8][nr].y, acc[mr][nr], 0, 0, 0);
          }
          {
            constexpr int MPK = MR * NR * 2, LPK = NR + MR, EACH = MPK / LPK, REM = MPK - EACH * LPK;
#pragma unroll
            for (int k8 = 0; k8 < KC8; ++k8) {
#pragma unroll
              for (int j = 0; j < NR; ++j) {
                __builtin_amdgcn_sched_group_barrier(0x020, 1, 0);
                __builtin_amdgcn_sched_group_barrier(0x008, EACH, 0);
              }
#pragma unroll
              for (int j = 0; j < MR; ++j) {
                __builtin_amdgcn_sched_group_barrier(0x100, 1, 0);
                __builtin_amdgcn_sched_group_barrier(0x008, EACH, 0);
              }
              if (REM > 0) __builtin_amdgcn_sched_group_barrier(0x008, REM, 0);
            }
          }
        }
      }
    } else if constexpr (BREG) {
#pragma unroll
      for (int tp = 0; tp < G::NT; ++tp) {
        const int dz = tp / (G::KH * G::KW), dy = (tp / G::KW) % G::KH, dx = tp % G::KW;
        const int toff = ((dz * G::PY + dy) * G::PX + dx) * S2;
        float2 ac[KC8][MR];
#pragma unroll
        for (int k8 = 0; k8 < KC8; ++k8)
#pragma unroll
          for (int mr = 0; mr < MR; ++mr) ac[k8][mr] = lds2[abase[mr] + toff + k8 * 4];
#pragma unroll
        for (int k8 = 0; k8 < KC8; ++k8) {
#pragma unroll
          for (int mr = 0; mr < MR; ++mr)
#pragma unroll
            for (int nr = 0; nr < NR; ++nr)
              acc[mr][nr] = __builtin_amdgcn_mfma_f32_16x16x4f32(ac[k8][mr].x, breg[tp][k8][nr].x, acc[mr][nr], 0, 0, 0);
#pragma unroll
          for (int mr = 0; mr < MR; ++mr)
#pragma unroll
            for (int nr = 0; nr < NR; ++nr)
              acc[mr][nr] = __builtin_amdgcn_mfma_f32_16x16x4f32(ac[k8][mr].y, breg[tp][k8][nr].y, acc[mr][nr], 0, 0, 0);
        }
      }
    } else {
      int koff[KC8];
#pragma unroll
      for (int k8 = 0; k8 < KC8; ++k8)
        koff[k8] = min((c0 >> 3) + k8, nkc8_total - 1) * nb16_total * 64;
      if constexpr (TAPPAIR) {
        constexpr int NP = (G::NT + 1) / 2;
        typedef unsigned int wu4 __attribute__((ext_vector_type(4)));
        auto wload4 = [&](int idx4, int nr) __attribute__((always_inline)) -> float4 {
          const wu4 v = __builtin_amdgcn_raw_buffer_load_b128(wrs, wvo[nr] * 2, idx4 * 16, 0);
          return make_float4(__uint_as_float(v.x), __uint_as_float(v.y), __uint_as_float(v.z), __uint_as_float(v.w));
        };
        float4 b4[KC8][NR];
#pragma unroll
        for (int k8 = 0; k8 < KC8; ++k8)
#pragma unroll
          for (int nr = 0; nr < NR; ++nr) b4[k8][nr] = wload4(koff[k8], nr);
#pragma unroll
        for (int p = 0; p < NP; ++p) {
          constexpr int KHW = G::KH * G::KW;
          const int t0 = 2 * p, t1 = min(2 * p + 1, G::NT - 1);
          const int o0 = (((t0 / KHW) * G::PY + (t0 / G::KW) % G::KH) * G::PX + t0 % G::KW) * S2;
          const int o1 = (((t1 / KHW) * G::PY + (t1 / G::KW) % G::KH) * G::PX + t1 % G::KW) * S2;
          float2 a0[KC8][MR], a1[KC8][MR];
          float4 bc[KC8][NR];
#pragma unroll
          for (int k8 = 0; k8 < KC8; ++k8)
#pragma unroll
            for (int mr = 0; mr < MR; ++mr) {
              a0[k8][mr] = lds2[abase[mr] + o0 + k8 * 4];
              a1[k8][mr] = lds2[abase[mr] + o1 + k8 * 4];
            }
          const int wn = min(p + 1, NP - 1) * tap_stride;
#pragma unroll
          for (int k8 = 0; k8 < KC8; ++k8)
#pragma unroll
            for (int nr = 0; nr < NR; ++nr) {
              bc[k8][nr] = b4[k8][nr];
              b4[k8][nr] = wload4(wn + koff[k8], nr);
            }
#define JH_TP_STEP(AV, AC, BC)                                                                              \
  _Pragma("unroll") for (int mr = 0; mr < MR; ++mr) _Pragma("unroll") for (int nr = 0; nr < NR; ++nr)     \
    acc[mr][nr] = __builtin_amdgcn_mfma_f32_16x16x4f32(AV[k8][mr].AC, bc[k8][nr].BC, acc[mr][nr], 0, 0, 0);
#pragma unroll
          for (int k8 = 0; k8 < KC8; ++k8) { JH_TP_STEP(a0, x, x) JH_TP_STEP(a0, y, y) }
#pragma unroll
          for (int k8 = 0; k8 < KC8; ++k8) { JH_TP_STEP(a1, x, z) JH_TP_STEP(a1, y, w) }
#undef JH_TP_STEP
        }
      } else {
      float2 bn[KC8][NR];
#pragma unroll
      for (int k8 = 0; k8 < KC8; ++k8)
#pragma unroll
        for (int nr = 0; nr < NR; ++nr) bn[k8][nr] = wload(koff[k8], nr);
      int tap = 0;
      for (int dz = 0; dz < G::KD; ++dz)
        for (int dy = 0; dy < G::KH; ++dy) {
          const int row_off = (dz * G::PY + dy) * G::PX * S2;
#pragma unroll
          for (int dx = 0; dx < G::KW; ++dx, ++tap) {
            float2 bc[KC8][NR], ac[KC8][MR];
#pragma unroll
            for (int k8 = 0; k8 < KC8; ++k8)
#pragma unroll
              for (int mr = 0; mr < MR; ++mr) ac[k8][mr] = lds2[abase[mr] + row_off + dx * S2 + k8 * 4];
            const int wn = min(tap + 1, G::NT - 1) * tap_stride;
#pragma unroll
            for (int k8 = 0; k8 < KC8; ++k8)
#pragma unroll
              for (int nr = 0; nr < NR; ++nr) {
                bc[k8][nr] = bn[k8][nr];
                bn[k8][nr] = wload(wn + koff[k8], nr);
              }
#pragma unroll
            for (int k8 = 0; k8 < KC8; ++k8) {
#pragma unroll
              for (int mr = 0; mr < MR; ++mr)
#pragma unroll
                for (int nr = 0; nr < NR; ++nr)
                  acc[mr][nr] = __builtin_amdgcn_mfma_f32_16x16x4f32(ac[k8][mr].x, bc[k8][nr].x, acc[mr][nr], 0, 0, 0);
#pragma unroll
              for (int mr = 0; mr < MR; ++mr)
#pragma unroll
                for (int nr = 0; nr < NR; ++nr)
                  acc[mr][nr] = __builtin_amdgcn_mfma_f32_16x16x4f32(ac[k8][mr].y, bc[k8][nr].y, acc[mr][nr], 0, 0, 0);
            }
          }
        }
      }
    }
  }

  __syncthreads();
  EpilogueArgs e;
  e.y = a.y + (size_t)n * a.Dy * a.Hy * a.Wy * a.cout_p;
  e.bias = a.bias;
  e.stats = a.stats ? a.stats + (size_t)n * a.cout_p * kStatW : nullptr;
  e.Dout = a.Dout; e.Hout = a.Hout; e.Wout = a.Wout; e.Hy = a.Hy; e.Wy = a.Wy;
  e.cout_p = a.cout_p; e.cout_p16 = a.cout_p16; e.os = a.ostride; e.osz = a.ostride;
  e.offz = a.phase[ph].ooff[0]; e.offy = a.phase[ph].ooff[1]; e.offx = a.phase[ph].ooff[2];
  if (oz0 + TZ <= a.Dout && oy0 + TY <= a.Hout && ox0 + TX <= a.Wout)
    conv_epilogue<MR, NR, TY, TX, 4, true>(acc, e, lds, nb0, oz0, oy0, ox0, tid);
  else
    conv_epilogue<MR, NR, TY, TX>(acc, e, lds, nb0, oz0, oy0, ox0, tid);
}

inline int pick_kc8(int cin_p, size_t (*lds_bytes)(int), size_t budget) {
  int best = 1;
  double best_cost = 1e30;
  for (int k = 1; k <= 4; ++k) {
    if (lds_bytes(k * 8) > budget && k > 1) continue;
    const int chunks = (cin_p + k * 8 - 1) / (k * 8);
    const double cost = (double)chunks * k * 8 / cin_p + 0.02 * chunks;
    if (cost < best_cost - 1e-9) { best_cost = cost; best = k; }
  }
  return best;
}

template <int ND, int K, int STRIDE, int TZ, int TY, int TX, int NRV, int KC8V>
int launch_conv_inst(const ConvArgs& b, dim3 grid, hipStream_t s) {
  using G = ConvGeom<ND, K, STRIDE, TZ, TY, TX>;
  size_t lds = G::lds_bytes(KC8V * 8);
  const size_t red = (size_t)4 * 4 * 16 * 2 * sizeof(double);
  if (lds < red) lds = red;
  lds += (size_t)b.nrm_floats * sizeof(float);
  JH_REQUIRE(lds <= 160 * 1024, "conv patch does not fit LDS");
  auto kern = conv_mfma_kernel<ND, K, STRIDE, TZ, TY, TX, NRV, KC8V>;
  static bool big_lds_enabled = false;
  if (lds > 64 * 1024 && !big_lds_enabled) {
    JH_CHECK_HIP(hipFuncSetAttribute(reinterpret_cast<const void*>(kern),
                                     hipFuncAttributeMaxDynamicSharedMemorySize, 160 * 1024));
    big_lds_enabled = true;
  }
  ConvArgs c = b;
  c.fgx = make_fastdiv(grid.x); c.fgy = make_fastdiv(grid.y);
  c.ftx = make_fastdiv((b.Wout + TX - 1) / TX); c.fty = make_fastdiv((b.Hout + TY - 1) / TY);
  JH_REQUIRE(b.nphase == 1 || b.nphase == 4 || b.nphase == 8, "phase count");
  hipLaunchKernelGGL(kern, grid, dim3(256), lds, s, c);
  JH_CHECK_HIP(hipGetLastError());
  return 0;
}

template <int ND, int K, int STRIDE, int TZ, int TY, int TX>
int launch_conv_geom(const ConvArgs& a, int nr, size_t lds_budget, hipStream_t s) {
  using G = ConvGeom<ND, K, STRIDE, TZ, TY, TX>;
  ConvArgs b = a;
  const int kc8 = pick_kc8(b.cin_p, &G::lds_bytes, lds_budget);
  b.kc = kc8 * 8;
  const int tiles = ((b.Dout + TZ - 1) / TZ) * ((b.Hout + TY - 1) / TY) * ((b.Wout + TX - 1) / TX);
  const int nb = b.cout_p16 / 16;
  while (nr > 1 && (long)tiles * ((nb + nr - 1) / nr) * b.N * b.nphase <= 128) --nr;
  dim3 grid(tiles, (nb + nr - 1) / nr, b.N * b.nphase);
#define JH_CONV_CASE(NRV, KV) \
  if (nr == NRV && kc8 == KV) return launch_conv_inst<ND, K, STRIDE, TZ, TY, TX, NRV, KV>(b, grid, s);
#define JH_CONV_ROW(NRV) JH_CONV_CASE(NRV, 1) JH_CONV_CASE(NRV, 2) JH_CONV_CASE(NRV, 3) JH_CONV_CASE(NRV, 4)
  JH_CONV_ROW(1) JH_CONV_ROW(2) JH_CONV_ROW(3) JH_CONV_ROW(4)
#undef JH_CONV_ROW
#undef JH_CONV_CASE
  JH_REQUIRE(false, "bad (NR, KC8)");
}

bool conv_pw_direct_eligible(const ConvDesc& d, const ConvArgs& a);
int launch_conv_pw_direct(const ConvArgs& a, hipStream_t s);

int launch_deconv4_fused(const ConvArgs& a, hipStream_t s);
bool deconv4_eligible(int cin_p, int cout_p16);

int conv_launch_2d_k1(const ConvArgs& a, int nr, int small, size_t budget, hipStream_t s);
int conv_launch_2d_k1_flat(const ConvArgs& a, int nr, size_t budget, hipStream_t s);
int conv_launch_2d_k2(const ConvArgs& a, int nr, int small, size_t budget, hipStream_t s);
int conv_launch_2d_k3(const ConvArgs& a, int stride, int nr, int small, size_t budget, hipStream_t s);
int conv_launch_2d_k3_w20(const ConvArgs& a, int nr, size_t budget, hipStream_t s);
int conv_launch_2d_k5(const ConvArgs& a, int stride, int nr, int small, size_t budget, hipStream_t s);
int conv_launch_2d_k5_w40(const ConvArgs& a, int stride, int nr, size_t budget, hipStream_t s);
int conv_launch_2d_k3s2_w20(const ConvArgs& a, int nr, size_t budget, hipStream_t s);
int conv_launch_2d_big(const ConvArgs& a, int k, int stride, int nr, size_t budget, hipStream_t s);
int conv_launch_3d_k1(const ConvArgs& a, int nr, int small, size_t budget, hipStream_t s);
int conv_launch_3d_k2s2(const ConvArgs& a, int nr, int small, size_t budget, hipStream_t s);
int conv_launch_3d_k3(const ConvArgs& a, int stride, int nr, int small, size_t budget, hipStream_t s);

}
```

jarvis-hybridnet_amd/csrc/deconv4.hip:

```cpp
#include <type_traits>
#include "conv_mfma.h"

namespace jh {

namespace {
constexpr int kDTY = 8, kDTX = 16, kDPY = kDTY + 2, kDPX = kDTX + 2, kDNPIX = kDPY * kDPX;
constexpr int kDSPAD = 4;
}

template <int NRP, int KC8, bool TR>
__global__ __launch_bounds__(256) void deconv4_fused_kernel(const ConvArgs a) {
  constexpr int MR = 2, NR = 4 * NRP;
  constexpr int KC = KC8 * 8, S = KC + kDSPAD, S2 = S / 2, Q4 = KC / 4, KP = KC8 / 2;
  static_assert(KC8 % 2 == 0 && S2 % 2 == 0, "paired operand layout");
  extern __shared__ __attribute__((aligned(16))) float lds_all[];
  float* nrm = lds_all;
  float* lds = lds_all + a.nrm_floats;
  float2* lds2 = reinterpret_cast<float2*>(lds);
  const int tid = threadIdx.x;
  const int lane = tid & 63;
  const int wave = __builtin_amdgcn_readfirstlane(tid >> 6);
  const int mrow = lane & 15, kq = lane >> 4;
  const int tiles_x = (a.Win + kDTX - 1) / kDTX;
  const BlockId bid = xcd_block();
  const int tile_x = bid.x % tiles_x, tile_y = bid.x / tiles_x;
  const int n = bid.z;
  const int oy0 = tile_y * kDTY, ox0 = tile_x * kDTX;
  const int iy0 = oy0 - 1, ix0 = ox0 - 1;

  int abase[MR];
#pragma unroll
  for (int mr = 0; mr < MR; ++mr) {
    const int p = (wave * MR + mr) * 16 + mrow;
    abase[mr] = ((p / kDTX) * kDPX + p % kDTX) * S2 + kq * 2;
  }
  f32x4 acc[MR][NR];
#pragma unroll
  for (int mr = 0; mr < MR; ++mr)
#pragma unroll
    for (int nr = 0; nr < NR; ++nr) acc[mr][nr] = (f32x4){0.f, 0.f, 0.f, 0.f};

  if (a.in_stats) {
    for (int c = tid; c < a.cin_p; c += 256) {
      const double* st = a.in_stats + ((size_t)n * a.cin_p + c) * kStatW;
      const double mu = exact_read(st) * (double)a.in_inv;
      double var = exact_read(st + kLimbs) * (double)a.in_inv - mu * mu;
      if (var < 0.0) var = 0.0;
      nrm[c] = (float)mu;
      nrm[a.cin_p + c] = (float)(1.0 / sqrt(var + 1e-5));
    }
  }
  const float* __restrict__ xin = a.x + (size_t)n * a.Hin * a.Win * a.in_px;
  const int nkc8_total = a.cin_p >> 3;
  const float4* __restrict__ wbase = reinterpret_cast<const float4*>(a.w);
  const unsigned ulane = lane;
  const int tap_stride = (nkc8_total >> 1) * NRP * 64;
  const int phase_stride4 = (int)(a.phase_stride >> 2);

  constexpr int ITER = (kDNPIX * Q4 + 255) / 256;
  static_assert(256 % Q4 == 0, "one channel quad per thread");
  typedef float cf4 __attribute__((ext_vector_type(4)));
  float4 pf[ITER];
  int pvo[ITER];
  const __amdgpu_buffer_rsrc_t xrs = __builtin_amdgcn_make_buffer_rsrc(
      const_cast<float*>(xin), 0, (int)((size_t)a.Hin * a.Win * a.in_px * 4), 0x00020000);
  const int c4 = tid % Q4;
#pragma unroll
  for (int it = 0; it < ITER; ++it) {
    const int pix = tid / Q4 + it * (256 / Q4);
    const int px = pix % kDPX, py = pix / kDPX;
    const int iy = iy0 + py, ix = ix0 + px;
    const bool ok = pix < kDNPIX && iy >= 0 && iy < a.Hin && ix >= 0 && ix < a.Win;
    pvo[it] = ok ? ((iy * a.Win + ix) * a.in_px + c4 * 4) * 4 : (int)0x80000000;
  }
  auto issue_pf = [&](int c0) __attribute__((always_inline)) {
#pragma unroll
    for (int it = 0; it < ITER; ++it) {
      const int off = (c0 + c4 * 4 < a.in_px) ? pvo[it] : (int)0x80000000;
      const cf4 v = __builtin_bit_cast(cf4, __builtin_amdgcn_raw_buffer_load_b128(xrs, off, c0 * 4, 0));
      pf[it] = make_float4(v[0], v[1], v[2], v[3]);
    }
  };
  issue_pf(0);

  for (int c0 = 0; c0 < a.cin_p; c0 += KC) {
    __syncthreads();
    {
      const int mode = !a.in_stats ? 0 : (a.in_act == ACT_RELU ? 2 : (a.in_act == ACT_SILU ? 3 : 1));
      auto commit_pf = [&](auto mode_c) __attribute__((always_inline)) {
        constexpr int MODE = decltype(mode_c)::value;
        float4 mu = make_float4(0.f, 0.f, 0.f, 0.f), rs = make_float4(1.f, 1.f, 1.f, 1.f);
        const int cc = min(c0 + c4 * 4, a.cin_p - 4);
        if (MODE != 0) {
          mu = *reinterpret_cast<const float4*>(nrm + cc);
          rs = *reinterpret_cast<const float4*>(nrm + a.cin_p + cc);
        }
#pragma unroll
        for (int it = 0; it < ITER; ++it) {
          const int pix = tid / Q4 + it * (256 / Q4);
          if (pix < kDNPIX) {
            float4 v = pf[it];
            if (MODE != 0) {
              const float m = (pvo[it] < 0 || c0 + c4 * 4 >= a.in_px) ? 0.f : 1.f;
              v.x = (v.x - mu.x) * rs.x; v.y = (v.y - mu.y) * rs.y;
              v.z = (v.z - mu.z) * rs.z; v.w = (v.w - mu.w) * rs.w;
              if (MODE == 2) {
                v.x = fmaxf(v.x, 0.f); v.y = fmaxf(v.y, 0.f); v.z = fmaxf(v.z, 0.f); v.w = fmaxf(v.w, 0.f);
              } else if (MODE == 3) {
                v.x = silu_fast(v.x); v.y = silu_fast(v.y);
                v.z = silu_fast(v.z); v.w = silu_fast(v.w);
              }
              v.x *= m; v.y *= m; v.z *= m; v.w *= m;
            }
            float2* dst = lds2 + pix * S2 + (c4 >> 2) * 8 + (c4 & 1) * 4 + ((c4 >> 1) & 1);
            dst[0] = make_float2(v.x, v.y);
            dst[2] = make_float2(v.z, v.w);
          }
        }
      };
      if (mode == 0) commit_pf(std::integral_constant<int, 0>{});
      else if (mode == 3) commit_pf(std::integral_constant<int, 3>{});
      else if (mode == 2) commit_pf(std::integral_constant<int, 2>{});
      else commit_pf(std::integral_constant<int, 1>{});
    }
    __syncthreads();
    if (c0 + KC < a.cin_p) issue_pf(c0 + KC);

    int koff[KP];
#pragma unroll
    for (int k8 = 0; k8 < KP; ++k8) koff[k8] = min((c0 >> 4) + k8, (nkc8_total >> 1) - 1) * NRP * 64;
    auto wptr = [&](int g) __attribute__((always_inline)) -> const float4* {
      int idx = 0;
      for (int r = 0; r < 3; ++r)
        for (int s = 0; s < 3; ++s)
          for (int py = 0; py < 2; ++py)
            for (int px = 0; px < 2; ++px) {
              const int ty = r - py, tx = s - px;
              if (ty < 0 || ty > 1 || tx < 0 || tx > 1) continue;
              if (idx == g) return wbase + (size_t)(py * 2 + px) * phase_stride4 + (ty * 2 + tx) * tap_stride;
              ++idx;
            }
      return wbase;
    };
    float4 bq[3][KP][NRP];
#pragma unroll
    for (int g0 = 0; g0 < 2; ++g0) {
      const float4* w0 = wptr(g0) + ulane;
#pragma unroll
      for (int k8 = 0; k8 < KP; ++k8)
#pragma unroll
        for (int nr = 0; nr < NRP; ++nr) bq[g0][k8][nr] = w0[koff[k8] + nr * 64];
    }
    float4 an[KP][MR];
#pragma unroll
    for (int k8 = 0; k8 < KP; ++k8)
#pragma unroll
      for (int mr = 0; mr < MR; ++mr) an[k8][mr] = *reinterpret_cast<const float4*>(lds2 + abase[mr] + k8 * 8);
    int g = 0;
#pragma unroll
    for (int r = 0; r < 3; ++r)
#pragma unroll
      for (int s = 0; s < 3; ++s) {
        float4 ac[KP][MR];
#pragma unroll
        for (int k8 = 0; k8 < KP; ++k8)
#pragma unroll
          for (int mr = 0; mr < MR; ++mr) ac[k8][mr] = an[k8][mr];
        if (r * 3 + s + 1 < 9) {
          const int r1 = (r * 3 + s + 1) / 3, s1 = (r * 3 + s + 1) % 3;
#pragma unroll
          for (int k8 = 0; k8 < KP; ++k8)
#pragma unroll
            for (int mr = 0; mr < MR; ++mr)
              an[k8][mr] = *reinterpret_cast<const float4*>(lds2 + abase[mr] + (r1 * kDPX + s1) * S2 + k8 * 8);
        }
#pragma unroll
        for (int py = 0; py < 2; ++py)
#pragma unroll
          for (int px = 0; px < 2; ++px) {
            const int ty = r - py, tx = s - px;
            if (ty < 0 || ty > 1 || tx < 0 || tx > 1) continue;
            if (g + 2 < 16) {
              const float4* wn = wptr(g + 2) + ulane;
#pragma unroll
              for (int k8 = 0; k8 < KP; ++k8)
#pragma unroll
                for (int nr = 0; nr < NRP; ++nr) bq[(g + 2) % 3][k8][nr] = wn[koff[k8] + nr * 64];
            }
            __builtin_amdgcn_sched_barrier(0);
            const int ph = py * 2 + px;
#pragma unroll
            for (int k8 = 0; k8 < KP; ++k8) {
#define JH_D4_STEP(C)                                                                                          \
  _Pragma("unroll") for (int mr = 0; mr < MR; ++mr) _Pragma("unroll") for (int nr = 0; nr < NRP; ++nr)       \
    acc[mr][ph * NRP + nr] = TR ? __builtin_amdgcn_mfma_f32_16x16x4f32(bq[g % 3][k8][nr].C, ac[k8][mr].C,    \
                                                                       acc[mr][ph * NRP + nr], 0, 0, 0)       \
                                : __builtin_amdgcn_mfma_f32_16x16x4f32(ac[k8][mr].C, bq[g % 3][k8][nr].C,    \
                                                                       acc[mr][ph * NRP + nr], 0, 0, 0);
              JH_D4_STEP(x) JH_D4_STEP(y) JH_D4_STEP(z) JH_D4_STEP(w)
#undef JH_D4_STEP
            }
            __builtin_amdgcn_sched_barrier(0);
            ++g;
          }
      }
  }

  __syncthreads();
  EpilogueArgs e;
  e.y = a.y + (size_t)n * a.Hy * a.Wy * a.cout_p;
  e.bias = a.bias;
  e.stats = a.stats ? a.stats + (size_t)n * a.cout_p * kStatW : nullptr;
  e.Dout = 1; e.Hout = a.Hin; e.Wout = a.Win; e.Hy = a.Hy; e.Wy = a.Wy;
  e.cout_p = a.cout_p; e.cout_p16 = a.cout_p16; e.os = 2; e.osz = 2; e.offz = 0;
  const bool full = oy0 + kDTY <= a.Hin && ox0 + kDTX <= a.Win;
#pragma unroll
  for (int ph = 0; ph < 4; ++ph) {
    f32x4 pa[MR][NRP];
#pragma unroll
    for (int mr = 0; mr < MR; ++mr)
#pragma unroll
      for (int nr = 0; nr < NRP; ++nr) pa[mr][nr] = acc[mr][ph * NRP + nr];
    e.offy = ph >> 1; e.offx = ph & 1;
    if constexpr (TR) {
      if (full) conv_epilogue_tr<MR, NRP, kDTY, kDTX, true>(pa, e, 0, 0, oy0, ox0, tid);
      else conv_epilogue_tr<MR, NRP, kDTY, kDTX, false>(pa, e, 0, 0, oy0, ox0, tid);
    } else {
      if (full) conv_epilogue<MR, NRP, kDTY, kDTX, 4, true>(pa, e, lds, 0, 0, oy0, ox0, tid);
      else conv_epilogue<MR, NRP, kDTY, kDTX>(pa, e, lds, 0, 0, oy0, ox0, tid);
      if (e.stats && ph < 3) __syncthreads();
    }
  }
}

template <int NRP, int KC8, bool TR>
static int launch_deconv4_tr(const ConvArgs& a, hipStream_t s) {
  size_t lds = (size_t)kDNPIX * (KC8 * 8 + kDSPAD) * sizeof(float);
  const size_t red = (size_t)4 * 4 * 16 * 2 * sizeof(double);
  if (lds < red) lds = red;
  lds += (size_t)a.nrm_floats * sizeof(float);
  auto kern = deconv4_fused_kernel<NRP, KC8, TR>;
  const int tiles = ((a.Hin + kDTY - 1) / kDTY) * ((a.Win + kDTX - 1) / kDTX);
  hipLaunchKernelGGL(kern, dim3(tiles, 1, a.N), dim3(256), lds, s, a);
  JH_CHECK_HIP(hipGetLastError());
  return 0;
}

template <int NRP, int KC8>
static int launch_deconv4_inst(const ConvArgs& a, hipStream_t s) {
  if (!a.stats) return launch_deconv4_tr<NRP, KC8, true>(a, s);
  return launch_deconv4_tr<NRP, KC8, false>(a, s);
}

bool deconv4_eligible(int cin_p, int cout_p16) {
  return cout_p16 <= 32 && cin_p % 16 == 0;
}

int launch_deconv4_fused(const ConvArgs& a, hipStream_t s) {
  const int nrp = a.cout_p16 / 16;
  if (a.gate || nrp > 2 || a.nphase != 4) return -1;
  if (!a.paired) return -1;
  const int kc8 = a.cin_p % 32 == 0 ? 4 : 2;
  if (nrp == 2 && kc8 == 4) return launch_deconv4_inst<2, 4>(a, s);
  if (nrp == 2 && kc8 == 2) return launch_deconv4_inst<2, 2>(a, s);
  if (nrp == 1 && kc8 == 4) return launch_deconv4_inst<1, 4>(a, s);
  return launch_deconv4_inst<1, 2>(a, s);
}

}
```

jarvis-hybridnet_amd/csrc/jh_common.h:

```cpp
#pragma once
#include <hip/hip_runtime.h>
#include <cstdlib>
#include <cstdint>
#include <cstdio>
#include <string>
#include <vector>

namespace jh {

constexpr int kWave = 64;

#define JH_ENV_KNOB(name) ([]() -> int { static const int v = [] { const char* e = getenv(name); return e ? atoi(e) : -1; }(); return v; }())

inline int round_up(int v, int m) { return (v + m - 1) / m * m; }
inline int cpad(int c) { return round_up(c, 8); }

void set_error(const std::string& msg);
#define JH_CHECK_HIP(expr)                                                     \
  do {                                                                         \
    hipError_t _e = (expr);                                                    \
    if (_e != hipSuccess) {                                                    \
      jh::set_error(std::string(#expr) + ": " + hipGetErrorString(_e));        \
      return 1;                                                                \
    }                                                                          \
  } while (0)
#define JH_REQUIRE(cond, msg)                                                  \
  do {                                                                         \
    if (!(cond)) {                                                             \
      jh::set_error(std::string("requirement failed: ") + #cond + " (" + msg + \
                    ")");                                                      \
      return 1;                                                                \
    }                                                                          \
  } while (0)

struct Act {
  float* p = nullptr;
  int N = 0, D = 1, H = 0, W = 0, C = 0, Cp = 0;
  size_t pixels() const { return (size_t)D * H * W; }
  size_t elems() const { return (size_t)N * pixels() * Cp; }
  size_t bytes() const { return elems() * sizeof(float); }
};

struct HeatLayout {
  int cams_per_block = 0;
  size_t block_stride = 0, frame_stride = 0;
};

enum ActKind { ACT_NONE = 0, ACT_RELU = 1, ACT_SILU = 2 };

struct ProfRec { std::string name; double flops, bytes; hipEvent_t e0, e1; float ms; };
struct Profiler {
  bool on = false;
  std::vector<ProfRec> recs;
  void begin(const std::string& name, double flops, double bytes, hipStream_t s);
  void end(hipStream_t s);
  int finish();
};
Profiler& profiler();

struct ConvPhase {
  int pad[3];
  int ooff[3];
};

struct ConvDesc {
  int nd;
  int k;
  int stride;
  int ostride;
  int nphase;
  ConvPhase phase[8];
  int cin, cout;
  int latency_class;
};

struct ConvWeights {
  float* w = nullptr;
  int paired = 0;
  float* bias = nullptr;
  size_t phase_stride = 0;
  int cin_p = 0, cout_p16 = 0;
};

struct FastDiv {
  unsigned mul = 1, shift = 0, d = 1;
};
inline FastDiv make_fastdiv(unsigned d) {
  FastDiv f;
  f.d = d;
  unsigned l = 0;
  while ((1ull << l) < d) ++l;
  f.shift = l;
  f.mul = (unsigned)((((1ull << l) - d) << 32) / d + 1);
  return f;
}

struct SeGate {
  const double* pool = nullptr;
  const float *wr = nullptr, *br = nullptr, *we = nullptr, *be = nullptr;
  int C = 0, S = 0;
  float inv_hw = 0.f;
};

struct ConvArgs {
  const float* x;
  float* y;
  const float* w;
  const float* bias;
  const float* gate;
  SeGate se;
  const double* in_stats;
  float in_inv;
  int in_act;
  int nrm_floats;
  double* stats;
  int N, Din, Hin, Win, cin_p;
  int Dout, Hout, Wout;
  int Dy, Hy, Wy, cout_p;
  int cout_p16;
  int kc;
  int in_px;
  int ostride, nphase;
  int paired = 0;
  FastDiv fgx, fgy, ftx, fty;
  size_t phase_stride;
  ConvPhase phase[8];
};

int pack_conv_weights(const ConvDesc& d, const float* w_host, const float* b_host,
                      bool transposed, ConvWeights* out);
void free_conv_weights(ConvWeights* w);

struct InNorm {
  const double* stats = nullptr;
  float inv = 0.f;
  int act = 0;
};
int launch_conv(const ConvDesc& d, const ConvWeights& w, const Act& x, const Act& y,
                const float* gate, double* stats, hipStream_t s, const InNorm* in = nullptr,
                const SeGate* se = nullptr);
void conv_out_shape(const ConvDesc& d, int D, int H, int W, int* Do, int* Ho, int* Wo);

ConvDesc conv_desc(int nd, int k, int stride, int pad, int cin, int cout);
ConvDesc deconv2d_k4s2p1_desc(int cin, int cout);
ConvDesc deconv3d_k2s2_desc(int cin, int cout);

int launch_norm_apply(const Act& x, const double* stats, double eps, int act,
                      const float* r1, const float* r2, float* y, double* pool,
                      hipStream_t s, const double* r1_stats = nullptr, int min_block_kb = 0);
int launch_se_gate(const double* pool, int N, int C, int Cp, int S, float inv_hw,
                   const float* wr, const float* br, const float* we, const float* be,
                   float* gate, hipStream_t s);
bool depthwise_can_pool(int H, int W);
int launch_depthwise(const Act& x, const float* w, int k, float* y, double* stats,
                     hipStream_t s, double* pool = nullptr);
enum FuseMode { FUSE_SAME = 0, FUSE_UP2 = 1, FUSE_UP4 = 2, FUSE_POOL2 = 3 };
struct FuseArgs {
  const float* in[3];
  int mode[3];
  float w[3];
  int n_in;
  int act;
};
int launch_fuse(const FuseArgs& f, const Act& out, hipStream_t s);
int launch_maxpool2(const Act& x, float* y, hipStream_t s);

struct BlockId { unsigned x, y, z; };

constexpr int kLimbs = 3;
constexpr int kStatW = 2 * kLimbs;
#if defined(__HIPCC__)
__device__ __forceinline__ void exact_add(double* dst, double p) {
  const double h = rint(p * 0x1p-16) * 0x1p16;
  const double r = p - h;
  const double m = rint(r * 0x1p20) * 0x1p-20;
  const double l = rint((r - m) * 0x1p56) * 0x1p-56;
  if (h != 0.0) unsafeAtomicAdd(dst + 0, h);
  if (m != 0.0) unsafeAtomicAdd(dst + 1, m);
  if (l != 0.0) unsafeAtomicAdd(dst + 2, l);
}
__device__ __forceinline__ double exact_read(const double* src) { return (src[0] + src[1]) + src[2]; }
__device__ __forceinline__ void stat_add(double* st, float s1, float s2) {
  exact_add(st, (double)s1);
  exact_add(st + kLimbs, (double)s2);
}
__device__ __forceinline__ void exact_add_rounded(double* dst, double p) {
  const double a = fabs(p);
  double q;
  int slot;
  if (a < 0x1p5) { q = rint(p * 0x1p35) * 0x1p-35; slot = 2; }
  else if (a < 0x1p15) { q = rint(p * 0x1p25) * 0x1p-25; slot = 1; }
  else { q = rint(p * 0x1p15) * 0x1p-15; slot = 0; }
  if (q != 0.0) unsafeAtomicAdd(dst + slot, q);
}
__device__ __forceinline__ void stat_add(double* st, double s1, double s2) {
  exact_add_rounded(st, s1);
  exact_add_rounded(st + kLimbs, s2);
}
__device__ __forceinline__ void stat_acc(double& s1, double& s2, float v) {
  const double d = (double)v;
  s1 += d;
  s2 = fma(d, d, s2);
}
#endif

#if defined(__HIPCC__)
__device__ __forceinline__ unsigned xcd_linear(unsigned L, unsigned total) {
  const unsigned q = total >> 3, r = total & 7u, x = L & 7u, s = L >> 3;
  return x < r ? x * (q + 1) + s : r * (q + 1) + (x - r) * q + s;
}
__device__ __forceinline__ unsigned fd_div(unsigned x, const FastDiv& f) { return (__umulhi(x, f.mul) + x) >> f.shift; }
__device__ __forceinline__ BlockId xcd_block(const FastDiv& fgx, const FastDiv& fgy) {
  const unsigned gx = gridDim.x, gy = gridDim.y, gz = gridDim.z;
  const unsigned L = blockIdx.x + gx * (blockIdx.y + gy * blockIdx.z);
  const unsigned l = xcd_linear(L, gx * gy * gz);
  BlockId b;
  const unsigned l1 = fd_div(l, fgx);
  b.x = l - l1 * gx;
  b.z = fd_div(l1, fgy);
  b.y = l1 - b.z * gy;
  return b;
}
__device__ __forceinline__ BlockId xcd_block() {
  const unsigned gx = gridDim.x, gy = gridDim.y, gz = gridDim.z;
  const unsigned L = blockIdx.x + gx * (blockIdx.y + gy * blockIdx.z);
  unsigned l = xcd_linear(L, gx * gy * gz);
  BlockId b;
  b.x = l % gx; l /= gx;
  b.y = l % gy;
  b.z = l / gy;
  return b;
}
#endif

#if defined(__HIPCC__)
__device__ __forceinline__ float sum_xor16(float s) {
  const auto r = __builtin_amdgcn_permlane16_swap(__float_as_uint(s), __float_as_uint(s), false, false);
  return __uint_as_float(r[0]) + __uint_as_float(r[1]);
}
__device__ __forceinline__ float sum_xor32(float s) {
  const auto r = __builtin_amdgcn_permlane32_swap(__float_as_uint(s), __float_as_uint(s), false, false);
  return __uint_as_float(r[0]) + __uint_as_float(r[1]);
}
__device__ __forceinline__ double sum_xor16(double s) {
  const unsigned lo = (unsigned)__double2loint(s), hi = (unsigned)__double2hiint(s);
  const auto a = __builtin_amdgcn_permlane16_swap(lo, lo, false, false);
  const auto b = __builtin_amdgcn_permlane16_swap(hi, hi, false, false);
  return __hiloint2double((int)b[0], (int)a[0]) + __hiloint2double((int)b[1], (int)a[1]);
}
__device__ __forceinline__ double sum_xor32(double s) {
  const unsigned lo = (unsigned)__double2loint(s), hi = (unsigned)__double2hiint(s);
  const auto a = __builtin_amdgcn_permlane32_swap(lo, lo, false, false);
  const auto b = __builtin_amdgcn_permlane32_swap(hi, hi, false, false);
  return __hiloint2double((int)b[0], (int)a[0]) + __hiloint2double((int)b[1], (int)a[1]);
}
__device__ __forceinline__ float silu_fast(float v) { return v * __builtin_amdgcn_rcpf(1.f + __expf(-v)); }
#endif

struct NodeArgs;
int launch_bifpn_node(const NodeArgs& a, hipStream_t s);
int pack_wino_weights(int cin, int cout, const float* w, const float* b, ConvWeights* out);
int wino_variant_from_env();
int launch_conv3d_wino(const ConvWeights& w, const Act& x, const Act& y, double* stats, hipStream_t s,
                       const InNorm* in, int variant = 4, const int* tables = nullptr);
int pack_bf16x3_weights(int cin, int cout, const float* w, const float* b, ConvWeights* out);
int launch_conv3d_bf16x3(const ConvWeights& w, const Act& x, const Act& y, double* stats, hipStream_t s,
                         const InNorm* in);
int pack_deconv4_bf16x3_weights(int cin, int cout, const float* w, ConvWeights* out);
bool deconv4_bf16x3_eligible(int cout);
int launch_deconv4_bf16x3(const ConvWeights& w, const Act& x, const Act& y, hipStream_t s, const InNorm* in);
bool conv_bf16x3_eligible(const ConvDesc& d);
int pack_conv_bf16x3_weights(const ConvDesc& d, const float* w, const float* b, ConvWeights* out);
int launch_conv_bf16x3(const ConvDesc& d, const ConvWeights& w, const Act& x, const Act& y, double* stats,
                       hipStream_t s, const InNorm* in);
int precision_mode();
void set_precision_mode(int m);
void pack_stem_weights(const float* w_host, float* packed, int cout);
int launch_stem_conv(const Act& x, const float* w_dev, const Act& y, double* stats, hipStream_t s);
struct StemSource;
int launch_stem_conv_src(const StemSource& src, const Act& x, const float* w_dev, const Act& y, double* stats,
                         hipStream_t s);
int launch_deconv_c1(const Act& x, const double* stats, float inv_cnt, int in_act, const float* w,
                     const Act& y, hipStream_t s);

int launch_zero(void* p, size_t bytes, hipStream_t s);

int launch_to_channel_last(const float* src, const Act& dst, hipStream_t s);
int launch_from_channel_last(const Act& src, float* dst, hipStream_t s);

}
```

jarvis-hybridnet_amd/csrc/nets.hip:

```cpp
#include <cmath>
#include <cstring>
#include <cstdlib>
#include "nets.h"
#include "bifpn_node.h"
#include "conv3d_wino.h"

namespace jh {

Profiler& profiler() {
  static Profiler p;
  return p;
}
void Profiler::begin(const std::string& name, double flops, double bytes, hipStream_t s) {
  ProfRec r{name, flops, bytes, nullptr, nullptr, 0.f};
  (void)hipEventCreate(&r.e0);
  (void)hipEventCreate(&r.e1);
  (void)hipEventRecord(r.e0, s);
  recs.push_back(r);
}
void Profiler::end(hipStream_t s) { (void)hipEventRecord(recs.back().e1, s); }
int Profiler::finish() {
  JH_CHECK_HIP(hipDeviceSynchronize());
  for (auto& r : recs) {
    if (!r.e0) continue;
    JH_CHECK_HIP(hipEventElapsedTime(&r.ms, r.e0, r.e1));
    (void)hipEventDestroy(r.e0);
    (void)hipEventDestroy(r.e1);
    r.e0 = r.e1 = nullptr;
  }
  return 0;
}

Plan::~Plan() {
  for (void* p : owned_) (void)hipFree(p);
  for (auto& c : convs_) free_conv_weights(&c);
}

int Plan::alloc(void** p, size_t bytes) {
  JH_CHECK_HIP(hipMalloc(p, bytes));
  owned_.push_back(*p);
  bytes_ += bytes;
  return 0;
}

int Plan::new_act(int N, int D, int H, int W, int C, Act* out) {
  out->N = N; out->D = D; out->H = H; out->W = W; out->C = C; out->Cp = cpad(C);
  if (alloc(reinterpret_cast<void**>(&out->p), out->bytes())) return 1;
  JH_CHECK_HIP(hipMemset(out->p, 0, out->bytes()));
  return 0;
}

size_t Plan::scratch(size_t doubles) {
  const size_t off = arena_doubles_;
  arena_doubles_ += (doubles + 7) / 8 * 8;
  return off;
}

int Plan::finish() {
  if (arena_doubles_ == 0) arena_doubles_ = 8;
  return alloc(reinterpret_cast<void**>(&arena_), arena_doubles_ * sizeof(double));
}

static int g_precision = [] {
  const char* e = getenv("JH_PRECISION");
  if (!e) return 0;
  return std::string(e) == "bf16x3" ? 1 : (std::string(e) == "bf16x3_wide" ? 2 : 0);
}();
int precision_mode() { return g_precision; }
void set_precision_mode(int m) { g_precision = m; }

int Plan::run(hipStream_t s) {
  if (launch_zero(arena_, arena_doubles_ * sizeof(double), s)) return 1;
  Profiler& pf = profiler();
  for (auto& op : ops_) {
    if (pf.on) pf.begin(op.name, op.flops, op.bytes, s);
    if (op.fn(s)) return 1;
    if (pf.on) pf.end(s);
  }
  return 0;
}

int Plan::upload(const std::vector<float>& host, float** dev) {
  if (alloc(reinterpret_cast<void**>(dev), host.size() * sizeof(float))) return 1;
  JH_CHECK_HIP(hipMemcpy(*dev, host.data(), host.size() * sizeof(float), hipMemcpyHostToDevice));
  return 0;
}

int Plan::get(const ParamMap& pm, const std::string& key, size_t numel, const float** out) {
  auto it = pm.find(key);
  JH_REQUIRE(it != pm.end(), "missing parameter " + key);
  JH_REQUIRE(it->second.size() == numel, "wrong element count for parameter " + key);
  *out = it->second.data();
  return 0;
}

int Plan::add_conv(const ParamMap& pm, const ConvDesc& d, const std::string& wkey,
                   const std::string& bkey, bool transposed, const Act& x, const Act& y,
                   const float* gate, bool want_stats, size_t* stats_off, long in_stats_off,
                   float in_inv, int in_act, const SeGate* se, long se_pool_off) {
  size_t taps;
  if (d.ostride > 1) taps = (d.nd == 2) ? 16 : 8;
  else taps = (size_t)d.k * d.k * (d.nd == 3 ? d.k : 1);
  const float *w = nullptr, *b = nullptr;
  ConvDesc dd = d;
  dd.latency_class = norm_block_kb == 0 ? 1 : 0;
  if (get(pm, wkey, (size_t)d.cin * d.cout * taps, &w)) return 1;
  if (!bkey.empty() && get(pm, bkey, d.cout, &b)) return 1;
  bool wino = d.nd == 3 && d.k == 3 && d.stride == 1 && d.ostride == 1 && !transposed && !gate;
  if (const char* e = getenv("JH_WINO")) wino = wino && atoi(e) != 0;
  const int wino_variant = wino ? wino_variant_from_env() : 0;
  const bool b3 = wino && precision >= 1;
  const bool d4b = d.nd == 2 && d.ostride > 1 && transposed && !b && !want_stats && !gate &&
                   precision >= 1 && deconv4_bf16x3_eligible(d.cout);
  const bool xb = !wino && !d4b && !transposed && !gate && !se && conv_bf16x3_eligible(d) && x.Cp == cpad(d.cin) &&
                  (precision == 2 || (precision == 1 && d.nd == 3));
  ConvWeights cw;
  if (xb) {
    if (pack_conv_bf16x3_weights(d, w, b, &cw)) return 1;
  } else if (d4b) {
    if (pack_deconv4_bf16x3_weights(d.cin, d.cout, w, &cw)) return 1;
  } else if (b3) {
    if (pack_bf16x3_weights(d.cin, d.cout, w, b, &cw)) return 1;
  } else if (wino) {
    if (pack_wino_weights(d.cin, d.cout, w, b, &cw)) return 1;
  } else {
    if (pack_conv_weights(d, w, b, transposed, &cw)) return 1;
  }
  convs_.push_back(cw);
  bytes_ += cw.phase_stride * d.nphase * sizeof(float);
  size_t off = 0;
  if (want_stats) {
    off = scratch((size_t)y.N * y.Cp * kStatW);
    if (stats_off) *stats_off = off;
  }
  const double opix = (double)y.N * y.pixels();
  const double taps_per_out = (d.ostride > 1) ? (double)taps / d.nphase : (double)taps;
  const double flops = 2.0 * opix * d.cin * d.cout * taps_per_out;
  const double bytes = 4.0 * ((double)x.N * x.pixels() * d.cin + opix * d.cout + (double)d.cin * d.cout * taps);
  const int* wino_tiles = nullptr;
  if (wino && !b3) {
    const std::vector<int> tt = wino_tables(y.D, y.H, y.W, x.Cp);
    if (!tt.empty()) {
      void* dev = nullptr;
      if (alloc(&dev, tt.size() * sizeof(int))) return 1;
      JH_CHECK_HIP(hipMemcpy(dev, tt.data(), tt.size() * sizeof(int), hipMemcpyHostToDevice));
      wino_tiles = static_cast<const int*>(dev);
    }
  }
  char nm[96];
  snprintf(nm, sizeof nm, "conv%dd_k%ds%d%s_%dx%d@%d", d.nd, d.ostride > 1 ? (d.nd == 2 ? 4 : 2) : d.k,
           d.ostride > 1 ? 2 : d.stride, d.ostride > 1 ? (d4b ? "Tbf16x3" : "T") : (b3 || xb ? "bf16x3" : (wino ? "wino" : "")), d.cin, d.cout, y.W);
  push(nm, flops, bytes,
       [this, d = dd, cw, x, y, gate, want_stats, off, in_stats_off, in_inv, in_act, wino, wino_variant, b3, d4b, xb,
        wino_tiles, sev = se ? *se : SeGate(), se_pool_off](hipStream_t s) {
    InNorm in;
    if (in_stats_off >= 0) { in.stats = sc((size_t)in_stats_off); in.inv = in_inv; in.act = in_act; }
    SeGate seg = sev;
    if (se_pool_off >= 0) seg.pool = sc((size_t)se_pool_off);
    if (xb) return launch_conv_bf16x3(d, cw, x, y, want_stats ? sc(off) : nullptr, s, &in);
    if (d4b) return launch_deconv4_bf16x3(cw, x, y, s, &in);
    if (b3) return launch_conv3d_bf16x3(cw, x, y, want_stats ? sc(off) : nullptr, s, &in);
    if (wino) return launch_conv3d_wino(cw, x, y, want_stats ? sc(off) : nullptr, s, &in, wino_variant, wino_tiles);
    return launch_conv(d, cw, x, y, gate, want_stats ? sc(off) : nullptr, s, &in, se_pool_off >= 0 ? &seg : nullptr);
  });
  return 0;
}

void Plan::add_norm(const Act& x, size_t stats_off, int act, const float* r1, const float* r2,
                    float* y, long pool_off, long r1_stats_off) {
  const double el = (double)x.N * x.pixels() * x.C;
  push("norm_apply", 8.0 * el, 4.0 * el * (1 + (y ? 1 : 0) + (r1 ? 1 : 0) + (r2 ? 1 : 0)),
       [this, x, stats_off, act, r1, r2, y, pool_off, r1_stats_off](hipStream_t s) {
    return launch_norm_apply(x, sc(stats_off), 1e-5, act, r1, r2, y,
                             pool_off >= 0 ? sc((size_t)pool_off) : nullptr, s,
                             r1_stats_off >= 0 ? sc((size_t)r1_stats_off) : nullptr, norm_block_kb);
  });
}

namespace {
struct SizeSpec { double width, depth; int fpn, cells, head; };
const SizeSpec kSizes[3] = {{0.5, 0.5, 56, 3, 64}, {1.0, 1.0, 88, 4, 88}, {1.1, 1.2, 160, 6, 160}};
const int kStages[7][6] = {{3, 1, 32, 16, 1, 1}, {3, 2, 16, 24, 6, 2}, {5, 2, 24, 40, 6, 2},
                           {3, 3, 40, 80, 6, 2}, {5, 3, 80, 112, 6, 1}, {5, 4, 112, 192, 6, 2},
                           {3, 1, 192, 320, 6, 1}};
struct Block { int stage, k, stride, cin, cout, expand; };

int scale_ch(int c, double width) {
  const double f = c * width;
  int o = std::max(8, (int)(f + 4) / 8 * 8);
  if (o < 0.9 * f) o += 8;
  return o;
}

void trunk(int size, int* stem, std::vector<Block>* blocks, int taps[3]) {
  const SizeSpec& s = kSizes[size];
  std::vector<Block> all;
  for (int st = 0; st < 7; ++st) {
    const int cin = scale_ch(kStages[st][2], s.width), cout = scale_ch(kStages[st][3], s.width);
    const int rep = (int)std::ceil(s.depth * kStages[st][1]);
    for (int r = 0; r < rep; ++r)
      all.push_back({st, kStages[st][0], r == 0 ? kStages[st][5] : 1, r == 0 ? cin : cout, cout,
                     kStages[st][4]});
  }
  int seen = 0, nt = 0;
  for (size_t i = 0; i < all.size() && nt < 3; ++i)
    if (all[i].stride == 2 && seen++ >= 1) taps[nt++] = (int)i - 1;
  blocks->assign(all.begin(), all.begin() + taps[2] + 1);
  *stem = scale_ch(32, s.width);
}

void fuse_weights(const float* p, int n, float* w) {
  float r[3], sum = 0.f;
  for (int i = 0; i < n; ++i) { r[i] = p[i] > 0.f ? p[i] : 0.f; sum += r[i]; }
  for (int i = 0; i < n; ++i) w[i] = r[i] / (sum + 1e-4f);
}
}

void EffTrackPlan::materialise(Ref* x) {
  if (x->st < 0) return;
  add_norm(x->a, (size_t)x->st, x->act, nullptr, nullptr, x->a.p, -1);
  x->st = -1;
}

int EffTrackPlan::mbconv(const ParamMap& pm, const std::string& p, int stage, int k, int stride,
                         int cin, int cout, int expand, Ref* xin, Ref* outr) {
  const bool skip = (stride == 1 && cin == cout);
  if (skip || (stage >= 4 && expand == 1)) materialise(xin);
  const Ref xr = *xin;
  const Act& x = xr.a;
  Act* out = &outr->a;
  const int mid = cin * expand;
  const int squeeze = std::max(1, (int)(cin * 0.25));
  const int Ho = (x.H + 2 * (k / 2) - k) / stride + 1, Wo = (x.W + 2 * (k / 2) - k) / stride + 1;
  Act raw;
  if (new_act(x.N, 1, Ho, Wo, mid, &raw)) return 1;
  size_t st1 = 0;
  const size_t pool = scratch((size_t)raw.N * raw.Cp * kLimbs);
  bool pooled = false;
  if (stage < 4) {
    if (add_conv(pm, conv_desc(2, k, stride, k / 2, cin, mid), p + "_depthwise_conv.weight", "",
                 false, x, raw, nullptr, true, &st1, xr.st, xr.inv, xr.act)) return 1;
  } else {
    Act e = x;
    if (expand != 1) {
      if (new_act(x.N, 1, x.H, x.W, mid, &e)) return 1;
      if (add_conv(pm, conv_desc(2, 1, 1, 0, cin, mid), p + "_expand_conv.weight", "", false, x, e,
                   nullptr, false, nullptr, xr.st, xr.inv, xr.act)) return 1;
    }
    JH_REQUIRE(stride == 1, "depthwise stages are stride 1");
    const float* w = nullptr;
    if (get(pm, p + "_depthwise_conv.weight", (size_t)mid * k * k, &w)) return 1;
    std::vector<float> wt((size_t)k * k * raw.Cp, 0.f);
    for (int c = 0; c < mid; ++c)
      for (int t = 0; t < k * k; ++t) wt[(size_t)t * raw.Cp + c] = w[(size_t)c * k * k + t];
    float* wd = nullptr;
    if (upload(wt, &wd)) return 1;
    st1 = scratch((size_t)raw.N * raw.Cp * kStatW);
    pooled = depthwise_can_pool(Ho, Wo);
    push(std::string("depthwise_k") + std::to_string(k) + (pooled ? "pool" : ""), 2.0 * raw.N * raw.pixels() * mid * k * k,
         8.0 * raw.N * raw.pixels() * mid, [this, e, wd, k, raw, st1, pool, pooled](hipStream_t s) {
      return launch_depthwise(e, wd, k, raw.p, sc(st1), s, pooled ? sc(pool) : nullptr);
    });
  }
  if (!pooled) add_norm(raw, st1, ACT_SILU, nullptr, nullptr, nullptr, (long)pool);
  const float *wr, *br, *we, *be;
  if (get(pm, p + "_se_reduce.weight", (size_t)squeeze * mid, &wr)) return 1;
  if (get(pm, p + "_se_reduce.bias", squeeze, &br)) return 1;
  if (get(pm, p + "_se_expand.weight", (size_t)mid * squeeze, &we)) return 1;
  if (get(pm, p + "_se_expand.bias", mid, &be)) return 1;
  float *dwr, *dbr, *dwe, *dbe, *gate = nullptr;
  if (upload(std::vector<float>(wr, wr + (size_t)squeeze * mid), &dwr)) return 1;
  if (upload(std::vector<float>(br, br + squeeze), &dbr)) return 1;
  if (upload(std::vector<float>(we, we + (size_t)mid * squeeze), &dwe)) return 1;
  if (upload(std::vector<float>(be, be + mid), &dbe)) return 1;
  const float inv_hw = 1.f / (float)(Ho * Wo);
  const bool se_fused = raw.N <= 32;
  SeGate seg;
  seg.wr = dwr; seg.br = dbr; seg.we = dwe; seg.be = dbe; seg.C = mid; seg.S = squeeze; seg.inv_hw = inv_hw;
  if (!se_fused) {
    if (alloc(reinterpret_cast<void**>(&gate), (size_t)raw.N * raw.Cp * sizeof(float))) return 1;
    push("se_gate", 4.0 * raw.N * mid * squeeze, 8.0 * raw.N * mid,
         [this, pool, raw, mid, squeeze, inv_hw, dwr, dbr, dwe, dbe, gate](hipStream_t s) {
      return launch_se_gate(sc(pool), raw.N, mid, raw.Cp, squeeze, inv_hw, dwr, dbr, dwe, dbe, gate, s);
    });
  }
  if (new_act(x.N, 1, Ho, Wo, cout, out)) return 1;
  size_t st2 = 0;
  if (add_conv(pm, conv_desc(2, 1, 1, 0, mid, cout), p + "_project_conv.weight", "", false, raw,
               *out, gate, true, &st2, (long)st1, 1.f / (float)(Ho * Wo), ACT_SILU,
               se_fused ? &seg : nullptr, se_fused ? (long)pool : -1)) return 1;
  if (skip) {
    add_norm(*out, st2, ACT_NONE, x.p, nullptr, out->p, -1);
    outr->st = -1;
  } else {
    outr->st = (long)st2;
    outr->inv = 1.f / (float)(Ho * Wo);
    outr->act = ACT_NONE;
  }
  return 0;
}

int EffTrackPlan::lateral(const ParamMap& pm, const std::string& p, int cout, const Ref& xr,
                          Ref* out) {
  const Act& x = xr.a;
  if (new_act(x.N, 1, x.H, x.W, cout, &out->a)) return 1;
  size_t st = 0;
  if (add_conv(pm, conv_desc(2, 1, 1, 0, x.C, cout), p + ".0.weight", p + ".0.bias", false, x,
               out->a, nullptr, true, &st, xr.st, xr.inv, xr.act)) return 1;
  out->st = (long)st;
  out->inv = 1.f / (float)(x.H * x.W);
  return 0;
}

int EffTrackPlan::pool(const Ref& x, Ref* out) {
  if (new_act(x.a.N, 1, x.a.H / 2, x.a.W / 2, x.a.C, &out->a)) return 1;
  out->st = x.st;
  out->inv = x.inv;
  const Act a = x.a, o = out->a;
  push("maxpool2", 0, 5.0 * o.N * o.pixels() * o.C * 4,
       [a, o](hipStream_t s) { return launch_maxpool2(a, o.p, s); });
  return 0;
}

int EffTrackPlan::node(const ParamMap& pm, const std::string& cp, int n_in, const Ref* ins,
                       const int* modes, const float* w, int act, const Act& like, int cout,
                       Ref* out, Ref* pooled) {
  const int cin = like.C;
  const float* dwh = nullptr;
  if (get(pm, cp + "depthwise_conv.weight", (size_t)cin * 9, &dwh)) return 1;
  std::vector<float> wt((size_t)9 * like.Cp, 0.f);
  for (int c = 0; c < cin; ++c)
    for (int t = 0; t < 9; ++t) wt[(size_t)t * like.Cp + c] = dwh[(size_t)c * 9 + t];
  float* dwd = nullptr;
  if (upload(wt, &dwd)) return 1;
  const float *pwh = nullptr, *bh = nullptr;
  if (get(pm, cp + "pointwise_conv.weight", (size_t)cin * cout, &pwh)) return 1;
  if (get(pm, cp + "pointwise_conv.bias", cout, &bh)) return 1;
  ConvWeights cw;
  if (pack_conv_weights(conv_desc(2, 1, 1, 0, cin, cout), pwh, bh, false, &cw)) return 1;
  convs_.push_back(cw);
  if (new_act(like.N, 1, like.H, like.W, cout, &out->a)) return 1;
  const size_t st = scratch((size_t)like.N * out->a.Cp * kStatW);
  out->st = (long)st;
  out->inv = 1.f / (float)(like.H * like.W);
  NodeArgs a{};
  a.n_in = n_in; a.act = act;
  long sts[3] = {-1, -1, -1};
  double bytes = 4.0 * like.N * like.pixels() * cout;
  for (int i = 0; i < n_in; ++i) {
    a.in[i] = ins[i].a.p; a.mode[i] = modes[i]; a.w[i] = w[i]; a.inv_cnt[i] = ins[i].inv;
    sts[i] = ins[i].st;
    bytes += 4.0 * ins[i].a.N * ins[i].a.pixels() * cin;
  }
  a.dw = dwd; a.pw = cw.w; a.bias = cw.bias; a.y = out->a.p;
  a.N = like.N; a.H = like.H; a.W = like.W; a.Cp = like.Cp;
  a.cout_p = out->a.Cp; a.cout_p16 = cw.cout_p16;
  a.rows = node_rows == 0 && like.Cp >= 88 ? 2 : node_rows;
  if (pooled) {
    pooled->a = Act{};
    const bool same3 = n_in == 3 && modes[1] == FUSE_SAME && modes[2] == FUSE_SAME && (like.Cp == 160 || a.rows == 2 || bifpn_rows_ragged88(a));
    if ((n_in == 2 || same3) && act == ACT_SILU && out->a.Cp == like.Cp && like.H % 2 == 0 && bifpn_rows_eligible(a)) {
      if (new_act(like.N, 1, like.H / 2, like.W / 2, cout, &pooled->a)) return 1;
      pooled->st = (long)st; pooled->inv = out->inv; pooled->act = out->act;
      a.y_pool = pooled->a.p;
      bytes += 4.0 * like.N * pooled->a.pixels() * cout;
    }
  }
  const double px = (double)like.N * like.pixels();
  char nm[64];
  snprintf(nm, sizeof nm, "bifpn_node_%dx%d@%d", cin, cout, like.W);
  const long s0 = sts[0], s1 = sts[1], s2 = sts[2];
  push(nm, 2.0 * px * cin * (9.0 + cout), bytes, [this, a, s0, s1, s2, st](hipStream_t s) {
    NodeArgs b = a;
    b.st[0] = s0 >= 0 ? sc((size_t)s0) : nullptr;
    b.st[1] = s1 >= 0 ? sc((size_t)s1) : nullptr;
    b.st[2] = s2 >= 0 ? sc((size_t)s2) : nullptr;
    b.stats = sc(st);
    return launch_bifpn_node(b, s);
  });
  return 0;
}

void EffTrackPlan::set_stem_traffic(double bytes) {
  if (stem_op_ >= 0 && stem_op_ < (int)ops_.size()) ops_[stem_op_].bytes = bytes;
}

int EffTrackPlan::build(const ParamMap& pm, const std::string& pre, int size, int joints, int N,
                        int H, int W, bool want_res1) {
  JH_REQUIRE(size >= 0 && size < 3, "model size");
  JH_REQUIRE(H % 64 == 0 && W % 64 == 0, "image side must be a multiple of 64");
  const SizeSpec& ss = kSizes[size];
  J = joints;
  int stem, taps[3];
  std::vector<Block> blocks;
  trunk(size, &stem, &blocks, taps);

  if (new_act(N, 1, H, W, 3, &input)) return 1;
  input.Cp = 4;
  Ref x;
  if (new_act(N, 1, H / 2, W / 2, stem, &x.a)) return 1;
  size_t st = 0;
  const std::string bb = pre + "backbone_net.model.";
  JH_REQUIRE(stem == 16 || stem == 32, "stem channels");
  const float* wh = nullptr;
  if (get(pm, bb + "_conv_stem.weight", (size_t)stem * 27, &wh)) return 1;
  std::vector<float> packed(27 * stem);
  pack_stem_weights(wh, packed.data(), stem);
  float* wd = nullptr;
  if (upload(packed, &wd)) return 1;
  st = scratch((size_t)N * stem * kStatW);
  const Act xin = input, xo = x.a;
  const double opix = (double)N * xo.pixels();
  stem_op_ = (int)ops_.size();
  stem_ch_ = stem;
  push("stem_conv_k3s2_3x" + std::to_string(stem) + "@" + std::to_string(xo.W), 2.0 * opix * 27 * stem,
       4.0 * ((double)N * xin.pixels() * 3 + opix * stem + 27 * stem),
       [this, xin, xo, wd, st](hipStream_t s) {
         if (stem_src.mode) return launch_stem_conv_src(stem_src, xin, wd, xo, sc(st), s);
         return launch_stem_conv(xin, wd, xo, sc(st), s);
       });
  const char* fuse = getenv("JH_STEM_FUSE");
  stem_fusable = !(fuse && atoi(fuse) == 0);
  x.st = (long)st;
  x.inv = 1.f / (float)((H / 2) * (W / 2));
  x.act = ACT_SILU;
  std::vector<Ref> outs(blocks.size() + 1);
  outs[0] = x;
  for (size_t i = 0; i < blocks.size(); ++i) {
    const Block& b = blocks[i];
// ... 164 lines not shown
```

Before: 2115 multi-view frames/s.

## Add window-form kernel for 2D stride-2 deconvolution computing all four phases per input window

Adds a new deconv4 path that packs weights so that each input window tile produces all four output sub-pixel phases in one pass, with the phases laid out as extra output columns. Each staged input tile is then reused across phases instead of being reloaded per phase, and separate edge blocks handle the last row and column. The path is enabled by default (JH_DECONV4_WINDOW=1) for layers with plain outputs (no stats, gate or SE) and certain channel counts. The shared input staging is factored into a helper struct, and a launch counter is exposed. Costs include extra template instantiations, more register pressure from triple-buffered weights, and an 0xFF memset in the op test path to catch unwritten outputs.

```diff
diff --git a/include/jarvis_hip.h b/include/jarvis_hip.h
--- a/include/jarvis_hip.h
+++ b/include/jarvis_hip.h
@@ -207,6 +207,7 @@
 int jh_op_conv(int nd, int kind, int k, int stride, int pad, int cin, int cout,
                const float* w_host, const float* b_host, const float* x_dev, int n, int d, int h,
                int w, const float* gate_dev, int norm_act, float* y_dev, void* stream);
+long jh_deconv4_window_launches(void);
 int jh_op_depthwise(int k, int c, const float* w_host, const float* x_dev, int n, int h, int w,
                     int norm_act, float* y_dev, void* stream);
 int jh_op_depthwise_pool(int k, int c, const float* w_host, const float* x_dev, int n, int h, int w,
diff --git a/jarvis-hybridnet_amd/_native.py b/jarvis-hybridnet_amd/_native.py
--- a/jarvis-hybridnet_amd/_native.py
+++ b/jarvis-hybridnet_amd/_native.py
@@ -153,6 +153,7 @@
     "jh_predictor_hybridnet_forward": (c_int, [c_void_p] * 9),
     "jh_op_conv": (c_int, [c_int] * 7 + [c_void_p, c_void_p, c_void_p] + [c_int] * 4 +
                    [c_void_p, c_int, c_void_p, c_void_p]),
+    "jh_deconv4_window_launches": (ctypes.c_long, []),
     "jh_op_depthwise": (c_int, [c_int, c_int, c_void_p, c_void_p, c_int, c_int, c_int, c_int,
                                 c_void_p, c_void_p]),
     "jh_op_depthwise_pool": (c_int, [c_int, c_int, c_void_p, c_void_p, c_int, c_int, c_int, c_void_p, c_void_p,
diff --git a/jarvis-hybridnet_amd/csrc/api.hip b/jarvis-hybridnet_amd/csrc/api.hip
--- a/jarvis-hybridnet_amd/csrc/api.hip
+++ b/jarvis-hybridnet_amd/csrc/api.hip
@@ -1144,12 +1144,15 @@
   return 0;
 }
 
+long jh_deconv4_window_launches(void) { return deconv4_window_launches(); }
+
 int jh_op_conv(int nd, int kind, int k, int stride, int pad, int cin, int cout,
                const float* w_host, const float* b_host, const float* x_dev, int n, int d, int h,
                int w, const float* gate_dev, int norm_act, float* y_dev, void* stream) {
   hipStream_t s = static_cast<hipStream_t>(stream);
   ConvDesc desc = kind == 0 ? conv_desc(nd, k, stride, pad, cin, cout)
                             : (kind == 1 ? deconv2d_k4s2p1_desc(cin, cout) : deconv3d_k2s2_desc(cin, cout));
+  desc.plain_out = norm_act < 0 && !gate_dev;
   Scratch sc;
   Act x, y;
   if (nd == 2) d = 1;
@@ -1157,7 +1160,7 @@
   int Do, Ho, Wo;
   conv_out_shape(desc, d, h, w, &Do, &Ho, &Wo);
   if (sc.act(n, Do, Ho, Wo, cout, &y)) return 1;
-  JH_CHECK_HIP(hipMemsetAsync(y.p, 0, y.bytes(), s));
+  JH_CHECK_HIP(hipMemsetAsync(y.p, kind == 1 && desc.plain_out ? 0xFF : 0, y.bytes(), s));
   bool wino = kind == 0 && nd == 3 && k == 3 && stride == 1 && pad == 1 && !gate_dev;
   if (const char* e = getenv("JH_WINO")) wino = wino && atoi(e) != 0;
   const bool b3 = wino && precision_mode() >= 1;
diff --git a/jarvis-hybridnet_amd/csrc/conv_host.hip b/jarvis-hybridnet_amd/csrc/conv_host.hip
--- a/jarvis-hybridnet_amd/csrc/conv_host.hip
+++ b/jarvis-hybridnet_amd/csrc/conv_host.hip
@@ -62,9 +62,16 @@
   const int nk8 = cin_p / 8, nb = cout_p16 / 16;
   const size_t phase_stride = (size_t)ntap * nk8 * nb * 128;
   std::vector<float> packed(phase_stride * d.nphase, 0.f);
-  const bool paired = d.nd == 2 && d.ostride > 1 && deconv4_eligible(cin_p, cout_p16);
+  const int cout_p = cpad(d.cout);
+  int wmode = 1;
+  if (const char* e = getenv("JH_DECONV4_WINDOW")) wmode = atoi(e);
+  const bool window = d.nd == 2 && d.ostride > 1 && d.plain_out && wmode != 0 &&
+                      deconv4_window_eligible(cin_p, cout_p, wmode >= 2);
+  const int npair = (nk8 + 1) / 2, nbw = (4 * cout_p + 15) / 16;
+  const bool paired = !window && d.nd == 2 && d.ostride > 1 && deconv4_eligible(cin_p, cout_p16);
   const bool tap_paired = d.nd == 3 && d.k == 3 && d.stride == 2 && d.ostride == 1;
   if (tap_paired) packed.assign((size_t)((ntap + 1) / 2) * nk8 * nb * 256, 0.f);
+  if (window) packed.assign((size_t)ntap * npair * nbw * 256, 0.f);
   int skd, sk;
   if (d.ostride > 1 && d.nd == 2) { skd = 1; sk = 4; }
   else if (d.ostride > 1 && d.nd == 3) { skd = 2; sk = 2; }
@@ -92,6 +99,12 @@
               const int lane = kq * 16 + nn;
               if (tap_paired)
                 packed[((((size_t)(tap / 2)) * nk8 + kc8) * nb + nbk) * 256 + lane * 4 + (tap & 1) * 2 + j] = v;
+              else if (window) {
+                const int sub = (1 - d.phase[ph].ooff[1]) * 2 + (1 - d.phase[ph].ooff[2]);
+                const int col = sub * cout_p + co;
+                packed[(((size_t)tap * npair + kc8 / 2) * nbw + col / 16) * 256 + (kq * 16 + col % 16) * 4 +
+                       (kc8 & 1) * 2 + j] = v;
+              }
               else if (paired)
                 packed[ph * phase_stride + (((size_t)tap * (nk8 / 2) + kc8 / 2) * nb + nbk) * 256 + lane * 4 + (kc8 & 1) * 2 + j] = v;
               else
@@ -99,8 +112,8 @@
             }
         }
   }
-  out->cin_p = cin_p; out->cout_p16 = cout_p16; out->paired = tap_paired ? 2 : (paired ? 1 : 0);
-  out->phase_stride = tap_paired ? packed.size() : phase_stride;
+  out->cin_p = cin_p; out->cout_p16 = cout_p16; out->paired = tap_paired ? 2 : (window ? 3 : (paired ? 1 : 0));
+  out->phase_stride = tap_paired ? packed.size() : (window ? packed.size() / d.nphase : phase_stride);
   JH_CHECK_HIP(hipMalloc(&out->w, packed.size() * sizeof(float)));
   JH_CHECK_HIP(hipMemcpy(out->w, packed.data(), packed.size() * sizeof(float), hipMemcpyHostToDevice));
   out->bias = nullptr;
@@ -165,7 +178,12 @@
   units *= (long)a.nphase * a.N;
   const int nr = pick_nr(w.cout_p16 / 16, taps, (in && in->stats && in->act == ACT_SILU) || gate || (se && se->pool),
                          units);
-  const size_t budget = 40 * 1024;
+  const size_t budget = kConvLdsBudget;
+  if (a.paired == 3) {
+    JH_REQUIRE(d.nd == 2 && d.ostride == 2 && d.k == 2 && !stats && !gate && !(se && se->pool),
+               "window-form weights on a layer with statistics or a gate");
+    return launch_deconv4_window(a, s);
+  }
   if (d.nd == 2 && d.ostride == 2 && d.k == 2) {
     const int rc = launch_deconv4_fused(a, s);
     if (rc >= 0) return rc;
diff --git a/jarvis-hybridnet_amd/csrc/conv_mfma.h b/jarvis-hybridnet_amd/csrc/conv_mfma.h
--- a/jarvis-hybridnet_amd/csrc/conv_mfma.h
+++ b/jarvis-hybridnet_amd/csrc/conv_mfma.h
@@ -606,6 +606,8 @@
     conv_epilogue<MR, NR, TY, TX>(acc, e, lds, nb0, oz0, oy0, ox0, tid);
 }
 
+constexpr size_t kConvLdsBudget = 40 * 1024;
+
 inline int pick_kc8(int cin_p, size_t (*lds_bytes)(int), size_t budget) {
   int best = 1;
   double best_cost = 1e30;
@@ -666,6 +668,8 @@
 
 int launch_deconv4_fused(const ConvArgs& a, hipStream_t s);
 bool deconv4_eligible(int cin_p, int cout_p16);
+int launch_deconv4_window(const ConvArgs& a, hipStream_t s);
+bool deconv4_window_eligible(int cin_p, int cout_p, bool wide);
 
 int conv_launch_2d_k1(const ConvArgs& a, int nr, int small, size_t budget, hipStream_t s);
 int conv_launch_2d_k1_flat(const ConvArgs& a, int nr, size_t budget, hipStream_t s);
diff --git a/jarvis-hybridnet_amd/csrc/deconv4.hip b/jarvis-hybridnet_amd/csrc/deconv4.hip
--- a/jarvis-hybridnet_amd/csrc/deconv4.hip
+++ b/jarvis-hybridnet_amd/csrc/deconv4.hip
@@ -1,3 +1,4 @@
+#include <atomic>
 #include <type_traits>
 #include "conv_mfma.h"
 
@@ -8,10 +9,95 @@
 constexpr int kDSPAD = 4;
 }
 
+__device__ __forceinline__ void deconv4_load_norm(const ConvArgs& a, float* nrm, int n, int tid) {
+  if (a.in_stats) {
+    for (int c = tid; c < a.cin_p; c += 256) {
+      const double* st = a.in_stats + ((size_t)n * a.cin_p + c) * kStatW;
+      const double mu = exact_read(st) * (double)a.in_inv;
+      double var = exact_read(st + kLimbs) * (double)a.in_inv - mu * mu;
+      if (var < 0.0) var = 0.0;
+      nrm[c] = (float)mu;
+      nrm[a.cin_p + c] = (float)(1.0 / sqrt(var + 1e-5));
+    }
+  }
+}
+
+template <int KC8, int NPIX>
+struct Deconv4Stage {
+  static constexpr int KC = KC8 * 8, S2 = (KC + kDSPAD) / 2, Q4 = KC / 4, ITER = (NPIX * Q4 + 255) / 256;
+  static_assert(256 % Q4 == 0, "one channel quad per thread");
+  typedef float cf4 __attribute__((ext_vector_type(4)));
+  float4 pf[ITER];
+  int pvo[ITER];
+  __amdgpu_buffer_rsrc_t xrs;
+  int tid, c4;
+
+  template <class Map>
+  __device__ __forceinline__ void init(const ConvArgs& a, const float* xin, int tid_, Map map) {
+    tid = tid_;
+    c4 = tid % Q4;
+    xrs = __builtin_amdgcn_make_buffer_rsrc(const_cast<float*>(xin), 0, (int)((size_t)a.Hin * a.Win * a.in_px * 4),
+                                            0x00020000);
+#pragma unroll
+    for (int it = 0; it < ITER; ++it) {
+      const int pix = tid / Q4 + it * (256 / Q4);
+      int iy = 0, ix = 0;
+      const bool ok = map(pix, &iy, &ix) && iy >= 0 && iy < a.Hin && ix >= 0 && ix < a.Win;
+      pvo[it] = ok ? ((iy * a.Win + ix) * a.in_px + c4 * 4) * 4 : (int)0x80000000;
+    }
+  }
+  __device__ __forceinline__ void issue(const ConvArgs& a, int c0) {
+#pragma unroll
+    for (int it = 0; it < ITER; ++it) {
+      const int off = (c0 + c4 * 4 < a.in_px) ? pvo[it] : (int)0x80000000;
+      const cf4 v = __builtin_bit_cast(cf4, __builtin_amdgcn_raw_buffer_load_b128(xrs, off, c0 * 4, 0));
+      pf[it] = make_float4(v[0], v[1], v[2], v[3]);
+    }
+  }
+  template <int MODE>
+  __device__ __forceinline__ void commit_mode(const ConvArgs& a, const float* nrm, float2* lds2, int c0) {
+    float4 mu = make_float4(0.f, 0.f, 0.f, 0.f), rs = make_float4(1.f, 1.f, 1.f, 1.f);
+    const int cc = min(c0 + c4 * 4, a.cin_p - 4);
+    if (MODE != 0) {
+      mu = *reinterpret_cast<const float4*>(nrm + cc);
+      rs = *reinterpret_cast<const float4*>(nrm + a.cin_p + cc);
+    }
+#pragma unroll
+    for (int it = 0; it < ITER; ++it) {
+      const int pix = tid / Q4 + it * (256 / Q4);
+      if (pix < NPIX) {
+        float4 v = pf[it];
+        if (MODE != 0) {
+          const float m = (pvo[it] < 0 || c0 + c4 * 4 >= a.in_px) ? 0.f : 1.f;
+          v.x = (v.x - mu.x) * rs.x; v.y = (v.y - mu.y) * rs.y;
+          v.z = (v.z - mu.z) * rs.z; v.w = (v.w - mu.w) * rs.w;
+          if (MODE == 2) {
+            v.x = fmaxf(v.x, 0.f); v.y = fmaxf(v.y, 0.f); v.z = fmaxf(v.z, 0.f); v.w = fmaxf(v.w, 0.f);
+          } else if (MODE == 3) {
+            v.x = silu_fast(v.x); v.y = silu_fast(v.y);
+            v.z = silu_fast(v.z); v.w = silu_fast(v.w);
+          }
+          v.x *= m; v.y *= m; v.z *= m; v.w *= m;
+        }
+        float2* dst = lds2 + pix * S2 + (c4 >> 2) * 8 + (c4 & 1) * 4 + ((c4 >> 1) & 1);
+        dst[0] = make_float2(v.x, v.y);
+        dst[2] = make_float2(v.z, v.w);
+      }
+    }
+  }
+  __device__ __forceinline__ void commit(const ConvArgs& a, const float* nrm, float2* lds2, int c0) {
+    const int mode = !a.in_stats ? 0 : (a.in_act == ACT_RELU ? 2 : (a.in_act == ACT_SILU ? 3 : 1));
+    if (mode == 0) commit_mode<0>(a, nrm, lds2, c0);
+    else if (mode == 3) commit_mode<3>(a, nrm, lds2, c0);
+    else if (mode == 2) commit_mode<2>(a, nrm, lds2, c0);
+    else commit_mode<1>(a, nrm, lds2, c0);
+  }
+};
+
 template <int NRP, int KC8, bool TR>
 __global__ __launch_bounds__(256) void deconv4_fused_kernel(const ConvArgs a) {
   constexpr int MR = 2, NR = 4 * NRP;
-  constexpr int KC = KC8 * 8, S = KC + kDSPAD, S2 = S / 2, Q4 = KC / 4, KP = KC8 / 2;
+  constexpr int KC = KC8 * 8, S = KC + kDSPAD, S2 = S / 2, KP = KC8 / 2;
   static_assert(KC8 % 2 == 0 && S2 % 2 == 0, "paired operand layout");
   extern __shared__ __attribute__((aligned(16))) float lds_all[];
   float* nrm = lds_all;
@@ -40,16 +126,7 @@
 #pragma unroll
     for (int nr = 0; nr < NR; ++nr) acc[mr][nr] = (f32x4){0.f, 0.f, 0.f, 0.f};
 
-  if (a.in_stats) {
-    for (int c = tid; c < a.cin_p; c += 256) {
-      const double* st = a.in_stats + ((size_t)n * a.cin_p + c) * kStatW;
-      const double mu = exact_read(st) * (double)a.in_inv;
-      double var = exact_read(st + kLimbs) * (double)a.in_inv - mu * mu;
-      if (var < 0.0) var = 0.0;
-      nrm[c] = (float)mu;
-      nrm[a.cin_p + c] = (float)(1.0 / sqrt(var + 1e-5));
-    }
-  }
+  deconv4_load_norm(a, nrm, n, tid);
   const float* __restrict__ xin = a.x + (size_t)n * a.Hin * a.Win * a.in_px;
   const int nkc8_total = a.cin_p >> 3;
   const float4* __restrict__ wbase = reinterpret_cast<const float4*>(a.w);
@@ -57,74 +134,18 @@
   const int tap_stride = (nkc8_total >> 1) * NRP * 64;
   const int phase_stride4 = (int)(a.phase_stride >> 2);
 
-  constexpr int ITER = (kDNPIX * Q4 + 255) / 256;
-  static_assert(256 % Q4 == 0, "one channel quad per thread");
-  typedef float cf4 __attribute__((ext_vector_type(4)));
-  float4 pf[ITER];
-  int pvo[ITER];
-  const __amdgpu_buffer_rsrc_t xrs = __builtin_amdgcn_make_buffer_rsrc(
-      const_cast<float*>(xin), 0, (int)((size_t)a.Hin * a.Win * a.in_px * 4), 0x00020000);
-  const int c4 = tid % Q4;
-#pragma unroll
-  for (int it = 0; it < ITER; ++it) {
-    const int pix = tid / Q4 + it * (256 / Q4);
-    const int px = pix % kDPX, py = pix / kDPX;
-    const int iy = iy0 + py, ix = ix0 + px;
-    const bool ok = pix < kDNPIX && iy >= 0 && iy < a.Hin && ix >= 0 && ix < a.Win;
-    pvo[it] = ok ? ((iy * a.Win + ix) * a.in_px + c4 * 4) * 4 : (int)0x80000000;
-  }
-  auto issue_pf = [&](int c0) __attribute__((always_inline)) {
-#pragma unroll
-    for (int it = 0; it < ITER; ++it) {
-      const int off = (c0 + c4 * 4 < a.in_px) ? pvo[it] : (int)0x80000000;
-      const cf4 v = __builtin_bit_cast(cf4, __builtin_amdgcn_raw_buffer_load_b128(xrs, off, c0 * 4, 0));
-      pf[it] = make_float4(v[0], v[1], v[2], v[3]);
-    }
-  };
-  issue_pf(0);
+  Deconv4Stage<KC8, kDNPIX> st;
+  st.init(a, xin, tid, [&](int pix, int* iy, int* ix) {
+    *iy = iy0 + pix / kDPX; *ix = ix0 + pix % kDPX;
+    return pix < kDNPIX;
+  });
+  st.issue(a, 0);
 
   for (int c0 = 0; c0 < a.cin_p; c0 += KC) {
     __syncthreads();
-    {
-      const int mode = !a.in_stats ? 0 : (a.in_act == ACT_RELU ? 2 : (a.in_act == ACT_SILU ? 3 : 1));
-      auto commit_pf = [&](auto mode_c) __attribute__((always_inline)) {
-        constexpr int MODE = decltype(mode_c)::value;
-        float4 mu = make_float4(0.f, 0.f, 0.f, 0.f), rs = make_float4(1.f, 1.f, 1.f, 1.f);
-        const int cc = min(c0 + c4 * 4, a.cin_p - 4);
-        if (MODE != 0) {
-          mu = *reinterpret_cast<const float4*>(nrm + cc);
-          rs = *reinterpret_cast<const float4*>(nrm + a.cin_p + cc);
-        }
-#pragma unroll
-        for (int it = 0; it < ITER; ++it) {
-          const int pix = tid / Q4 + it * (256 / Q4);
-          if (pix < kDNPIX) {
-            float4 v = pf[it];
-            if (MODE != 0) {
-              const float m = (pvo[it] < 0 || c0 + c4 * 4 >= a.in_px) ? 0.f : 1.f;
-              v.x = (v.x - mu.x) * rs.x; v.y = (v.y - mu.y) * rs.y;
-              v.z = (v.z - mu.z) * rs.z; v.w = (v.w - mu.w) * rs.w;
-              if (MODE == 2) {
-                v.x = fmaxf(v.x, 0.f); v.y = fmaxf(v.y, 0.f); v.z = fmaxf(v.z, 0.f); v.w = fmaxf(v.w, 0.f);
-              } else if (MODE == 3) {
-                v.x = silu_fast(v.x); v.y = silu_fast(v.y);
-                v.z = silu_fast(v.z); v.w = silu_fast(v.w);
-              }
-              v.x *= m; v.y *= m; v.z *= m; v.w *= m;
-            }
-            float2* dst = lds2 + pix * S2 + (c4 >> 2) * 8 + (c4 & 1) * 4 + ((c4 >> 1) & 1);
-            dst[0] = make_float2(v.x, v.y);
-            dst[2] = make_float2(v.z, v.w);
-          }
-        }
-      };
-      if (mode == 0) commit_pf(std::integral_constant<int, 0>{});
-      else if (mode == 3) commit_pf(std::integral_constant<int, 3>{});
-      else if (mode == 2) commit_pf(std::integral_constant<int, 2>{});
-      else commit_pf(std::integral_constant<int, 1>{});
-    }
+    st.commit(a, nrm, lds2, c0);
     __syncthreads();
-    if (c0 + KC < a.cin_p) issue_pf(c0 + KC);
+    if (c0 + KC < a.cin_p) st.issue(a, c0 + KC);
 
     int koff[KP];
 #pragma unroll
@@ -252,6 +273,220 @@
   return launch_deconv4_tr<NRP, KC8, false>(a, s);
 }
 
+namespace {
+constexpr int kWPY = kDTY + 1, kWPX = kDTX + 1, kWNPIX = kWPY * kWPX;
+constexpr int kWELINE = 130, kWEZERO = kWELINE, kWENPIX = kWELINE + 1;
+constexpr int kWLDSPIX = kWNPIX > kWENPIX ? kWNPIX : kWENPIX;
+}
+
+template <int NB, int KC8, bool EDGE>
+__device__ __forceinline__ void deconv4_window_body(const ConvArgs& a, const int n, const int unit) {
+  constexpr int MR = 2, NT = EDGE ? 3 : 4, NCH = NB / 2, NG = NT * NCH;
+  constexpr int KC = KC8 * 8, S = KC + kDSPAD, S2 = S / 2, KP = KC8 / 2;
+  constexpr int NPIX = EDGE ? kWENPIX : kWNPIX;
+  static_assert(KC8 % 2 == 0 && S2 % 2 == 0 && NB % 2 == 0, "paired operand layout, column blocks in twos");
+  extern __shared__ __attribute__((aligned(16))) float lds_all[];
+  float* nrm = lds_all;
+  float* lds = lds_all + a.nrm_floats;
+  float2* lds2 = reinterpret_cast<float2*>(lds);
+  const int tid = threadIdx.x;
+  const int lane = tid & 63;
+  const int wave = __builtin_amdgcn_readfirstlane(tid >> 6);
+  const int mrow = lane & 15, kq = lane >> 4;
+  const int H = a.Hin, W = a.Win;
+  const int tiles_x = (W + kDTX - 1) / kDTX;
+  const int wy0 = EDGE ? 0 : (unit / tiles_x) * kDTY, wx0 = EDGE ? 0 : (unit % tiles_x) * kDTX;
+  const int e0 = unit * 128;
+
+  int arow[NT][MR];
+#pragma unroll
+  for (int mr = 0; mr < MR; ++mr) {
+    const int p = (wave * MR + mr) * 16 + mrow;
+    if (EDGE) {
+      const int e = e0 + p;
+      const bool rw = e <= W, cw = !rw && e <= W + H;
+      arow[0][mr] = (rw ? p : (cw ? p + 1 : kWEZERO)) * S2 + kq * 2;
+      arow[1][mr] = (rw ? p + 1 : kWEZERO) * S2 + kq * 2;
+      arow[2][mr] = (cw ? p + 2 : kWEZERO) * S2 + kq * 2;
+    } else {
+#pragma unroll
+      for (int t = 0; t < NT; ++t)
+        arow[t][mr] = ((p / kDTX + (t >> 1)) * kWPX + p % kDTX + (t & 1)) * S2 + kq * 2;
+    }
+  }
+  f32x4 acc[MR][NB];
+#pragma unroll
+  for (int mr = 0; mr < MR; ++mr)
+#pragma unroll
+    for (int nb = 0; nb < NB; ++nb) acc[mr][nb] = (f32x4){0.f, 0.f, 0.f, 0.f};
+
+  deconv4_load_norm(a, nrm, n, tid);
+  const float* __restrict__ xin = a.x + (size_t)n * H * W * a.in_px;
+  const int npair = ((a.cin_p >> 3) + 1) >> 1;
+  const float4* __restrict__ wbase = reinterpret_cast<const float4*>(a.w);
+  const unsigned ulane = lane;
+  const int tap_stride = npair * NB * 64;
+
+  Deconv4Stage<KC8, NPIX> st;
+  st.init(a, xin, tid, [&](int pix, int* iy, int* ix) {
+    if (EDGE) {
+      const int pos = e0 + pix;
+      const bool row = pos <= W + 1;
+      *iy = row ? H - 1 : pos - W - 3;
+      *ix = row ? pos - 1 : W - 1;
+      return pix < kWELINE;
+    }
+    *iy = wy0 - 1 + pix / kWPX; *ix = wx0 - 1 + pix % kWPX;
+    return pix < kWNPIX;
+  });
+  st.issue(a, 0);
+
+  for (int c0 = 0; c0 < a.cin_p; c0 += KC) {
+    __syncthreads();
+    st.commit(a, nrm, lds2, c0);
+    __syncthreads();
+    if (c0 + KC < a.cin_p) st.issue(a, c0 + KC);
+
+    int koff[KP];
+#pragma unroll
+    for (int k8 = 0; k8 < KP; ++k8) koff[k8] = min((c0 >> 4) + k8, npair - 1) * NB * 64;
+    auto wptr = [&](int g) __attribute__((always_inline)) -> const float4* {
+      return wbase + (g / NCH) * tap_stride + (g % NCH) * 128;
+    };
+    float4 bq[3][KP][2];
+#pragma unroll
+    for (int g0 = 0; g0 < 2 && g0 < NG; ++g0) {
+      const float4* w0 = wptr(g0) + ulane;
+#pragma unroll
+      for (int k8 = 0; k8 < KP; ++k8)
+#pragma unroll
+        for (int nr = 0; nr < 2; ++nr) bq[g0][k8][nr] = w0[koff[k8] + nr * 64];
+    }
+    float4 an[KP][MR];
+#pragma unroll
+    for (int k8 = 0; k8 < KP; ++k8)
+#pragma unroll
+      for (int mr = 0; mr < MR; ++mr) an[k8][mr] = *reinterpret_cast<const float4*>(lds2 + arow[0][mr] + k8 * 8);
+    int g = 0;
+#pragma unroll
+    for (int t = 0; t < NT; ++t) {
+      float4 ac[KP][MR];
+#pragma unroll
+      for (int k8 = 0; k8 < KP; ++k8)
+#pragma unroll
+        for (int mr = 0; mr < MR; ++mr) ac[k8][mr] = an[k8][mr];
+      if (t + 1 < NT) {
+#pragma unroll
+        for (int k8 = 0; k8 < KP; ++k8)
+#pragma unroll
+          for (int mr = 0; mr < MR; ++mr)
+            an[k8][mr] = *reinterpret_cast<const float4*>(lds2 + arow[t + 1 < NT ? t + 1 : t][mr] + k8 * 8);
+      }
+#pragma unroll
+      for (int ch = 0; ch < NCH; ++ch) {
+        if (g + 2 < NG) {
+          const float4* wn = wptr(g + 2) + ulane;
+#pragma unroll
+          for (int k8 = 0; k8 < KP; ++k8)
+#pragma unroll
+            for (int nr = 0; nr < 2; ++nr) bq[(g + 2) % 3][k8][nr] = wn[koff[k8] + nr * 64];
+        }
+        __builtin_amdgcn_sched_barrier(0);
+#pragma unroll
+        for (int k8 = 0; k8 < KP; ++k8) {
+#define JH_D4W_STEP(C)                                                                                         \
+  _Pragma("unroll") for (int mr = 0; mr < MR; ++mr) _Pragma("unroll") for (int nr = 0; nr < 2; ++nr)          \
+    acc[mr][ch * 2 + nr] = __builtin_amdgcn_mfma_f32_16x16x4f32(bq[g % 3][k8][nr].C, ac[k8][mr].C,            \
+                                                                acc[mr][ch * 2 + nr], 0, 0, 0);
+          JH_D4W_STEP(x) JH_D4W_STEP(y) JH_D4W_STEP(z) JH_D4W_STEP(w)
+#undef JH_D4W_STEP
+        }
+        __builtin_amdgcn_sched_barrier(0);
+        ++g;
+      }
+    }
+  }
+
+  float* __restrict__ y = a.y + (size_t)n * a.Hy * a.Wy * a.cout_p;
+  const int cp = a.cout_p;
+#pragma unroll
+  for (int mr = 0; mr < MR; ++mr) {
+    const int p = (wave * MR + mr) * 16 + mrow;
+    int wy, wx;
+    bool ok;
+    if (EDGE) {
+      const int e = e0 + p;
+      const bool rw = e <= W;
+      wy = rw ? H : e - W - 1; wx = rw ? e : W;
+      ok = e <= W + H;
+    } else {
+      wy = wy0 + p / kDTX; wx = wx0 + p % kDTX;
+      ok = wy < H && wx < W;
+    }
+#pragma unroll
+    for (int nb = 0; nb < NB; ++nb) {
+      const int c = nb * 16 + kq * 4;
+      const int sub = (c >= cp) + (c >= 2 * cp) + (c >= 3 * cp);
+      const int ch = c - sub * cp;
+      const int oy = 2 * wy - 1 + (sub >> 1), ox = 2 * wx - 1 + (sub & 1);
+      f32x4 v = acc[mr][nb];
+      if (a.bias) v += *reinterpret_cast<const f32x4*>(a.bias + min(ch, a.cout_p16 - 4));
+      if (ok && c < 4 * cp && (unsigned)oy < (unsigned)a.Hy && (unsigned)ox < (unsigned)a.Wy)
+        *reinterpret_cast<f32x4*>(y + ((size_t)oy * a.Wy + ox) * cp + ch) = v;
+    }
+  }
+}
+
+template <int NB, int KC8>
+__global__ __launch_bounds__(256) void deconv4_window_kernel(const ConvArgs a) {
+  const BlockId bid = xcd_block();
+  const int tiles = ((a.Hin + kDTY - 1) / kDTY) * ((a.Win + kDTX - 1) / kDTX);
+  if ((int)bid.x < tiles) deconv4_window_body<NB, KC8, false>(a, bid.z, bid.x);
+  else deconv4_window_body<NB, KC8, true>(a, bid.z, bid.x - tiles);
+}
+
+static std::atomic<long> g_window_launches{0};
+long deconv4_window_launches() { return g_window_launches.load(); }
+
+static_assert(ConvGeom<2, 2, 1, 1, kDTY, kDTX>::NPIX * (32 + 4) * sizeof(float) <= kConvLdsBudget &&
+              ConvGeom<2, 2, 1, 1, 8, 8>::NPIX <= ConvGeom<2, 2, 1, 1, kDTY, kDTX>::NPIX,
+              "the general path's pass size must not depend on its tile geometry");
+static int deconv4_window_kc8(int cin_p) {
+  if (cin_p % 16 == 0) return cin_p % 32 == 0 ? 4 : 2;
+  const int k = pick_kc8(cin_p, &ConvGeom<2, 2, 1, 1, kDTY, kDTX>::lds_bytes, kConvLdsBudget);
+  return k % 2 == 0 ? k : 0;
+}
+
+bool deconv4_window_eligible(int cin_p, int cout_p, bool wide) {
+  const int nbw = (4 * cout_p + 15) / 16;
+  return (nbw == 2 || nbw == 6 || (wide && nbw == 8)) && cin_p % 8 == 0 && deconv4_window_kc8(cin_p) != 0;
+}
+
+template <int NB, int KC8>
+static int launch_deconv4_window_inst(const ConvArgs& a, hipStream_t s) {
+  const size_t lds = (size_t)kWLDSPIX * (KC8 * 8 + kDSPAD) * sizeof(float) + (size_t)a.nrm_floats * sizeof(float);
+  const int tiles = ((a.Hin + kDTY - 1) / kDTY) * ((a.Win + kDTX - 1) / kDTX);
+  const int edge = (a.Hin + a.Win + 1 + 127) / 128;
+  hipLaunchKernelGGL((deconv4_window_kernel<NB, KC8>), dim3(tiles + edge, 1, a.N), dim3(256), lds, s, a);
+  JH_CHECK_HIP(hipGetLastError());
+  ++g_window_launches;
+  return 0;
+}
+
+int launch_deconv4_window(const ConvArgs& a, hipStream_t s) {
+  const int nb = (4 * a.cout_p + 15) / 16, kc8 = deconv4_window_kc8(a.cin_p);
+  JH_REQUIRE(a.paired == 3 && a.nphase == 4 && !a.stats && !a.gate && !a.se.pool &&
+             deconv4_window_eligible(a.cin_p, a.cout_p, true), "not a layer of the window form");
+  JH_REQUIRE((long)a.Hin * a.Win * a.in_px < (1L << 29) && (long)a.Hy * a.Wy * a.cout_p < (1L << 31),
+             "image too large for the window form's 32-bit offsets");
+  if (nb == 8 && kc8 == 4) return launch_deconv4_window_inst<8, 4>(a, s);
+  if (nb == 8 && kc8 == 2) return launch_deconv4_window_inst<8, 2>(a, s);
+  if (nb == 6 && kc8 == 4) return launch_deconv4_window_inst<6, 4>(a, s);
+  if (nb == 6 && kc8 == 2) return launch_deconv4_window_inst<6, 2>(a, s);
+  if (nb == 2 && kc8 == 4) return launch_deconv4_window_inst<2, 4>(a, s);
+  return launch_deconv4_window_inst<2, 2>(a, s);
+}
+
 bool deconv4_eligible(int cin_p, int cout_p16) {
   return cout_p16 <= 32 && cin_p % 16 == 0;
 }
diff --git a/jarvis-hybridnet_amd/csrc/jh_common.h b/jarvis-hybridnet_amd/csrc/jh_common.h
--- a/jarvis-hybridnet_amd/csrc/jh_common.h
+++ b/jarvis-hybridnet_amd/csrc/jh_common.h
@@ -72,6 +72,7 @@
   ConvPhase phase[8];
   int cin, cout;
   int latency_class;
+  int plain_out;
 };
 
 struct ConvWeights {
@@ -144,6 +145,7 @@
 ConvDesc conv_desc(int nd, int k, int stride, int pad, int cin, int cout);
 ConvDesc deconv2d_k4s2p1_desc(int cin, int cout);
 ConvDesc deconv3d_k2s2_desc(int cin, int cout);
+long deconv4_window_launches();
 
 int launch_norm_apply(const Act& x, const double* stats, double eps, int act,
                       const float* r1, const float* r2, float* y, double* pool,
diff --git a/jarvis-hybridnet_amd/csrc/nets.hip b/jarvis-hybridnet_amd/csrc/nets.hip
--- a/jarvis-hybridnet_amd/csrc/nets.hip
+++ b/jarvis-hybridnet_amd/csrc/nets.hip
@@ -104,6 +104,7 @@
   const float *w = nullptr, *b = nullptr;
   ConvDesc dd = d;
   dd.latency_class = norm_block_kb == 0 ? 1 : 0;
+  dd.plain_out = !want_stats && !gate && !se;
   if (get(pm, wkey, (size_t)d.cin * d.cout * taps, &w)) return 1;
   if (!bkey.empty() && get(pm, bkey, d.cout, &b)) return 1;
   bool wino = d.nd == 3 && d.k == 3 && d.stride == 1 && d.ostride == 1 && !transposed && !gate;
@@ -124,7 +125,7 @@
   } else if (wino) {
     if (pack_wino_weights(d.cin, d.cout, w, b, &cw)) return 1;
   } else {
-    if (pack_conv_weights(d, w, b, transposed, &cw)) return 1;
+    if (pack_conv_weights(dd, w, b, transposed, &cw)) return 1;
   }
   convs_.push_back(cw);
   bytes_ += cw.phase_stride * d.nphase * sizeof(float);
```

Result: faster. 2141 multi-view frames/s, median of 6 (+1.3%).
